# genome/pindel

Hardware: AMD Instinct MI355X
Metric: one-end-anchored reads/sec through split-read search (close end + far end) (higher is better)
Workload: dtype u64; 1 GPU; BASELINE configs[2]: synthetic 10000000 x 100 bp one-end-anchored reads on a chr20-shaped reference (62435964 bp), all SV types (D/SI/TD/INV/none), Pindel defaults -x 2 -a 1 -m 3 -u 0.02 -e 0.01 -E 0.95 -H 8; reads_per_gpu=10000000, reads_total=10000000, read_len=100, insert_size=500, parallelism=reads sharded over 1 GPU(s) (weak scaling), reference replicated, no collective

## Files before the change

pindel_amd/csrc/pg_kernels.hip:

```cpp
#include <hip/hip_runtime.h>
#include <stdint.h>
#include <stdlib.h>

#include "pg_device.h"
#include "pg_lane_masks.h"
#include "pg_eval_masks.h"

typedef unsigned long long u64;
typedef unsigned int u32;
typedef u32 u32x4 __attribute__((ext_vector_type(4)));
typedef u32 u32x8 __attribute__((ext_vector_type(8)));

struct PgKArgs { PgDevRef ref; PgDevParams prm; PgDevBatch B; uint32_t max_len, levels; };
template <typename T> struct KaGlobal { static __device__ __forceinline__ T of(unsigned long long v) { return (T)v; } };
template <typename E> struct KaGlobal<E *> {
    static __device__ __forceinline__ E *of(unsigned long long v) { return (E *)(__attribute__((address_space(1))) E *)v; }
};
template <typename T>
__device__ __forceinline__ T karg_load(int off)
{
    const auto k = __builtin_amdgcn_kernarg_segment_ptr();
    if (sizeof(T) == 8) {
        unsigned long long v;
        asm volatile("s_load_dwordx2 %0, %1, %2\n\ts_waitcnt lgkmcnt(0)" : "=&s"(v) : "s"(k), "n"(off));
        return KaGlobal<T>::of(v);
    } else {
        unsigned int v;
        asm volatile("s_load_dword %0, %1, %2\n\ts_waitcnt lgkmcnt(0)" : "=&s"(v) : "s"(k), "n"(off));
        return (T)v;
    }
}
template <int OFF, typename T>
__device__ __forceinline__ void karg_load3(T &a, T &b, T &c)
{
    static_assert(sizeof(T) == 8, "pointers");
    const auto k = __builtin_amdgcn_kernarg_segment_ptr();
    unsigned long long x, y, z;
    asm volatile("s_load_dwordx2 %0, %3, %4\n\ts_load_dwordx2 %1, %3, %5\n\ts_load_dwordx2 %2, %3, %6\n\ts_waitcnt lgkmcnt(0)"
                 : "=&s"(x), "=&s"(y), "=&s"(z) : "s"(k), "n"(OFF), "n"(OFF + 8), "n"(OFF + 16));
    a = KaGlobal<T>::of(x); b = KaGlobal<T>::of(y); c = KaGlobal<T>::of(z);
}
#define KA(obj, member) karg_load<decltype(obj.member)>((int)offsetof(PgKArgs, obj.member))
#define KAP(member) karg_load<decltype(PgDevParams::member)>((int)offsetof(PgKArgs, prm.member))
#define PRM(member, dflt) (DEF ? (decltype(PgDevParams::member))(dflt) : KA(prm, member))
#define PG_DEF_MAX_RANGE_INDEX 2
#define PG_DEF_ADD_MM 1
#define PG_DEF_MIN_PERFECT 3
#define PG_DEF_MIN_CLOSE 8
#define PG_DEF_SPACER 100000u

#define WAVE 64
#define PG_N_XCD 8u
#define PG_WAVES(NB, Id) (sizeof(Lds<NB, Id>) <= 5120 ? 7 : (sizeof(Lds<NB, Id>) <= 6400 ? 6 : (sizeof(Lds<NB, Id>) <= 7680 ? 5 : 4)))
#define PG_BIG 0xffffu
#define PG_CHR_TAB 24
#define PG_PASS(nb) ((nb) >= 3 ? 32 : 64)
#define PG_CHR_TAB_N(nb) ((nb) >= 3 ? 0 : PG_CHR_TAB)
#define PG_MM_IN_WIN(nb) ((nb) <= 4)

__device__ __forceinline__ u64 ballot64(bool p) { return __builtin_amdgcn_ballot_w64(p); }
__device__ __forceinline__ bool lane_bit(u64 m) { return __builtin_amdgcn_inverse_ballot_w64(m); }
template <int N>
__device__ __forceinline__ u32 row_shr(u32 v)
{
    return (u32)__builtin_amdgcn_update_dpp(0, (int)v, 0x110 + N, 0xf, 0xf, true);
}
__device__ __forceinline__ u32 wave_shr1(u32 v)
{
    return (u32)__builtin_amdgcn_update_dpp(0, (int)v, 0x138, 0xf, 0xf, true);
}
__device__ __forceinline__ u64 wave_shr1(u64 v)
{
    return (u64)wave_shr1((u32)v) | ((u64)wave_shr1((u32)(v >> 32)) << 32);
}
__device__ __forceinline__ u32 wave_scan(u32 v)
{
    v += row_shr<1>(v);
    v += row_shr<2>(v);
    v += row_shr<4>(v);
    v += row_shr<8>(v);
    v += (u32)__builtin_amdgcn_update_dpp(0, (int)v, 0x142, 0xa, 0xf, false);
    v += (u32)__builtin_amdgcn_update_dpp(0, (int)v, 0x143, 0xc, 0xf, false);
    return v;
}
__device__ __forceinline__ u32 read_lane(u32 v, int l) { return (u32)__builtin_amdgcn_readlane((int)v, l); }
__device__ __forceinline__ u64 read_lane(u64 v, int l)
{
    return (u64)read_lane((u32)v, l) | ((u64)read_lane((u32)(v >> 32), l) << 32);
}

#define PG_SYNC()                                              \
    do {                                                       \
        __builtin_amdgcn_fence(__ATOMIC_RELEASE, "wavefront"); \
        __builtin_amdgcn_wave_barrier();                       \
        __builtin_amdgcn_fence(__ATOMIC_ACQUIRE, "wavefront"); \
    } while (0)
__device__ __forceinline__ int uni(int v) { return __builtin_amdgcn_readfirstlane(v); }
__device__ __forceinline__ int opaque(int v)
{
    asm volatile("" : "+v"(v));
    return v;
}
__device__ __forceinline__ int lane_now()
{
    return (int)__builtin_amdgcn_mbcnt_hi(~0u, __builtin_amdgcn_mbcnt_lo(~0u, (u32)opaque(0)));
}
__device__ __forceinline__ u64 low_bits(int n)
{
    return n >= 64 ? ~0ull : (n <= 0 ? 0ull : ((1ull << n) - 1ull));
}
__device__ __forceinline__ u32 low32(int n)
{
    return n >= 32 ? 0xffffffffu : (n <= 0 ? 0u : ((1u << n) - 1u));
}
__device__ __forceinline__ u32 low32_lane(int n)
{
    int t;
    asm("v_med3_i32 %0, %1, 0, 32" : "=v"(t) : "v"(n));
    u32 m;
    asm("v_bfm_b32 %0, %1, 0" : "=v"(m) : "v"(t));
    return m | (0u - ((u32)t >> 5));
}
__device__ __forceinline__ u32 low32_lane4(int n)
{
    int t, f;
    asm("v_med3_i32 %0, %1, 0, 32" : "=v"(t) : "v"(n));
    u32 m;
    asm("v_bfm_b32 %0, %1, 0" : "=v"(m) : "v"(t));
    asm("v_bfe_i32 %0, %1, 5, 1" : "=v"(f) : "v"(t));
    return m | (u32)f;
}
__device__ __forceinline__ u64 low_bits_lane(int n)
{
    return (u64)low32_lane4(n) | ((u64)low32_lane4(n - 32) << 32);
}
template <int NB, int NS, int mode, bool DEF, bool EXACT, int LEN>
constexpr bool pg_short_masks()
{
    if (!DEF || EXACT) return false;
    return !((NB == 4 && NS == 3 && mode == PG_MODE_FAR) || (NB == 8 && NS == 3 && mode == PG_MODE_CLOSE));
}
template <int NB, int NS, typename Id, int mode, bool DEF, bool EXACT, int LEN>
constexpr bool pg_short_eval()
{
    if (!DEF || EXACT) return false;
    if (LEN > 0) return true;
    return (NB == 3 && mode == PG_MODE_FAR) || (NB == 4 && NS == 4 && mode == PG_MODE_BOTH) || (NB == 8 && mode == PG_MODE_CLOSE);
}
__device__ __forceinline__ int count_below(u64 m)
{
    return (int)__builtin_amdgcn_mbcnt_hi((u32)(m >> 32), __builtin_amdgcn_mbcnt_lo((u32)m, 0u));
}
__device__ __forceinline__ u64 bit_range(int lo, int hi)
{
    return low_bits(hi) & ~low_bits(lo);
}
__device__ __forceinline__ u64 funnel64(u32 w0, u32 w1, u32 w2, u32 s)
{
    u32 a = __builtin_amdgcn_alignbit(w1, w0, s);
    u32 b = __builtin_amdgcn_alignbit(w2, w1, s);
    return (u64)a | ((u64)b << 32);
}
__device__ __forceinline__ u32 med3(u32 a, u32 b, u32 c)
{
    u32 r;
    asm("v_med3_u32 %0, %1, %2, %3" : "=v"(r) : "v"(a), "v"(b), "v"(c));
    return r;
}

template <int SHIFT, typename T>
__device__ __forceinline__ T *record_ptr(T *base, uint32_t rid)
{
    const u64 b = (u64)(uintptr_t)base;
    const u32 blo = (u32)uni((int)(u32)b), bhi = (u32)uni((int)(u32)(b >> 32)), r = (u32)uni((int)rid);
    u32 lo, hi;
    asm("s_lshl_b32 %0, %4, %5\n\ts_lshr_b32 %1, %4, %6\n\ts_add_u32 %0, %0, %2\n\ts_addc_u32 %1, %1, %3"
        : "=&s"(lo), "=&s"(hi) : "s"(blo), "s"(bhi), "s"(r), "n"(SHIFT), "n"(32 - SHIFT) : "scc");
    return KaGlobal<T *>::of((u64)lo | ((u64)hi << 32));
}

template <typename Id> struct IdFmt;
template <> struct IdFmt<u32> { static constexpr int RB = PG_REL_BITS_SMALL; };
template <> struct IdFmt<u64> { static constexpr int RB = PG_REL_BITS; };
template <typename Id>
__device__ __forceinline__ Id make_id(u32 rel, bool isB, u32 region)
{
    return (Id)rel | ((Id)(isB ? 1u : 0u) << IdFmt<Id>::RB) | ((Id)region << (IdFmt<Id>::RB + 1));
}

enum { QP_LO = 0, QP_HI = 1, QP_NN = 2, QP_OO = 3 };

template <int NB>
struct Query {
    const u64 *qp;
    bool allowF_, allowB_;
    bool cF_, cB_;
    bool first_ok_;
    bool o1_;
    __device__ __forceinline__ bool allowF() const { return allowF_; }
    __device__ __forceinline__ bool allowB() const { return allowB_; }
    __device__ __forceinline__ bool cF() const { return cF_; }
    __device__ __forceinline__ bool cB() const { return cB_; }
    __device__ __forceinline__ bool first_ok() const { return first_ok_; }
};
template <int NB> __device__ __forceinline__ u64 q_lo(const Query<NB> &Q, int b) { return Q.qp[QP_LO * NB + b]; }
template <int NB> __device__ __forceinline__ u64 q_hi(const Query<NB> &Q, int b) { return Q.qp[QP_HI * NB + b]; }
template <int NB> __device__ __forceinline__ u64 q_nn(const Query<NB> &Q, int b) { return Q.qp[QP_NN * NB + b]; }
template <int NB> __device__ __forceinline__ u64 q_oo(const Query<NB> &Q, int b) { return Q.qp[QP_OO * NB + b]; }

template <typename Id> struct AccB;
template <> struct AccB<u32> {
    typedef uint2 T;
    static __device__ __forceinline__ void load(const void *base, int i, u32 &m1, u32 &m2, u32 &ok, u32 &id)
    {
        const uint2 st = ((const uint2 *)base)[i];
        m1 = st.x & 0xffffu; m2 = (st.x >> 16) & 0x7fffu; ok = st.x >> 31; id = st.y;
    }
    static __device__ __forceinline__ void store(void *base, int i, u32 m1, u32 m2, u32 ok, u32 id)
    {
        const u32 c2 = m2 < 0x7fffu ? m2 : 0x7fffu;
        ((uint2 *)base)[i] = make_uint2(m1 | (c2 << 16) | (ok << 31), id);
    }
};
template <> struct AccB<u64> {
    typedef uint4 T;
    static __device__ __forceinline__ void load(const void *base, int i, u32 &m1, u32 &m2, u32 &ok, u64 &id)
    {
        const uint4 st = ((const uint4 *)base)[i];
        m1 = st.x; m2 = st.y & 0xffffu; ok = st.y >> 16; id = (u64)st.z | ((u64)st.w << 32);
    }
    static __device__ __forceinline__ void store(void *base, int i, u32 m1, u32 m2, u32 ok, u64 id)
    {
        ((uint4 *)base)[i] = make_uint4(m1, m2 | (ok << 16), (u32)id, (u32)(id >> 32));
    }
};

template <int NB, typename Id>
struct Lds {
    uint4 bufA[68];
    uint2 bufB[PG_PASS(NB) * NB];
    uint2 hdrB[64];
    u64 ringB[3 * NB];
    typename AccB<Id>::T accB[NB > 1 ? 64 * (NB - 1) : 1];
    u64 qp[2 * 4 * NB];
    uint16_t queue[PG_PASS(NB)];
    uint8_t mm_tab[PG_MM_IN_WIN(NB) ? 4 : 64 * NB + 64];
    uint2 chr_tab[PG_CHR_TAB_N(NB)];
#ifdef PG_TIMING
    u64 t_last;
    u32 t_acc[12];
    u32 t_pad[2];
#endif
    uint4 win[PG_WIN_STATIC_WORDS(NB)];
};

struct Search {
    int len, T, M, add_mm, bps, min_perfect, thr;
    uint16_t *queue;
    uint4 *win;
    uint4 *bufA;
    uint2 *bufB;
    uint2 *hdrB;
    u64 *ringB;
    void *accB;
    const uint8_t *mm_tab;
    const uint2 *chr_tab;
    u32 depth, jmask[2];
    u32 ro;
    u32 rid;
    u32 rp_lo, rp_hi;
    long long win_wo;
    int win_lo, win_hi, wbase;
    int nsurv;
    u32 nsurv_total;
#ifdef PG_TIMING
    u64 *t_last;
    u32 *t_acc;
    int t_base;
#define PG_T(S, k) do { if (threadIdx.x == 0) { const u64 t_ = __builtin_readcyclecounter(); (S).t_acc[k] += (u32)(t_ - *(S).t_last); *(S).t_last = t_; } } while (0)
#else
#define PG_T(S, k) ((void)0)
#endif
#ifdef PG_STOP
    u32 stopped;
#define PG_STOP_AT(S, k) do { asm volatile("s_nop 14\n\ts_nop %0\n\ts_nop %1" : : "n"((k) & 7), "n"((k) >> 3)); \
                              if (PG_STOP == (k) && uni(opaque(1))) { (S).stopped = 1u; return; } } while (0)
#define PG_STOPPED(S) do { if ((S).stopped) return; } while (0)
#define PG_STOP_AT_V(S, k, v) do { asm volatile("s_nop 14\n\ts_nop %0\n\ts_nop %1" : : "n"((k) & 7), "n"((k) >> 3)); \
                                 if (PG_STOP == (k) && uni(opaque(1))) { (S).stopped = 1u; return (v); } } while (0)
#define PG_STOPPED_V(S, v) do { if ((S).stopped) return (v); } while (0)
#else
#define PG_STOP_AT(S, k) ((void)0)
#define PG_STOPPED(S) ((void)0)
#define PG_STOP_AT_V(S, k, v) ((void)0)
#define PG_STOPPED_V(S, v) ((void)0)
#endif
#ifdef PG_DIAG
    u32 dg;
#endif
#if defined(PG_DIAG) && PG_DIAG == 2
#define PG_DG(S, sh) ((void)0)
#define PG_DC(S, sh) ((S).dg += 1u << (sh))
#define PG_DC_IF(S, cond, sh) ((S).dg += (cond) ? 1u << (sh) : 0u)
#elif defined(PG_DIAG)
#define PG_DG(S, sh) ((S).dg += 1u << (sh))
#define PG_DC(S, sh) ((void)0)
#define PG_DC_IF(S, cond, sh) ((void)0)
#else
#define PG_DG(S, sh) ((void)0)
#define PG_DC(S, sh) ((void)0)
#define PG_DC_IF(S, cond, sh) ((void)0)
#endif
    int cap_state;
    u32 sf;
    __device__ __forceinline__ bool want_cap() const { return (sf & 1u) != 0u; }
    __device__ __forceinline__ bool tierA() const { return (sf & 2u) != 0u; }
    __device__ __forceinline__ bool len_check() const { return (sf & 4u) != 0u; }
};

template <int NB, typename Id>
struct Acc {
    u32 m1, m2, ok;
    Id id;
    u32 a1, a2, aok;
    Id aid;
    u32 dirty;
    __device__ __forceinline__ void reset()
    {
        m1 = m2 = PG_BIG; ok = 0u; id = 0;
        a1 = a2 = PG_BIG; aok = 0u; aid = 0;
        dirty = 0u;
    }
};

template <typename Id>
__device__ __forceinline__ void fold(u32 &m1, u32 &m2, Id &id, u32 &ok, u32 k, Id cid, u32 okc)
{
    const bool lt = k < m1;
    m2 = med3(m1, m2, k);
    id = lt ? cid : id;
    ok = lt ? okc : ok;
    m1 = k < m1 ? k : m1;
}
template <typename Id>
__device__ __forceinline__ void merge(u32 &a1, u32 &a2, Id &aid, u32 &aok, u32 b1, u32 b2, Id bid, u32 bok)
{
    const bool lt = b1 < a1;
    const u32 hi1 = a1 > b1 ? a1 : b1, lo2 = a2 < b2 ? a2 : b2;
    a2 = hi1 < lo2 ? hi1 : lo2;
    aid = lt ? bid : aid;
    aok = lt ? bok : aok;
    a1 = lt ? b1 : a1;
}

__device__ __forceinline__ int max_mismatch_at(const u32 *mm_bp, int L)
{
    int m = 0;
#pragma unroll
    for (int k = 0; k < PG_MM_BREAKS; k++) m += (u32)L >= mm_bp[k] ? 1 : 0;
    return m;
}

template <int NB>
__device__ __forceinline__ long long chr_word_off_of(const PgDevRef &ref, const Search &S, int c)
{
    if (c < PG_CHR_TAB_N(NB)) {
        const uint2 e = S.chr_tab[c];
        if (uni((int)e.y) != 0) return (long long)(u64)(u32)uni((int)e.x);
    }
    const u64 w = KA(ref, chr_word_off)[c];
    return (long long)((u64)(u32)uni((int)(u32)w) | ((u64)(u32)uni((int)(u32)(w >> 32)) << 32));
}
template <int NB>
__device__ __forceinline__ int chr_size_of(const PgDevRef &ref, const Search &S, int c)
{
    if (c < PG_CHR_TAB_N(NB)) {
        const int sz = uni((int)S.chr_tab[c].y);
        if (sz != 0) return sz;
    }
    return uni((int)KA(ref, chr_size)[c]);
}

template <int NB>
__device__ __forceinline__ void block_masks(const Query<NB> &Q, int b, bool comp,
                                            u64 rlo, u64 rhi, u64 rnn, u64 &mis, u64 &qn)
{
    const u64 qlo = q_lo<NB>(Q, b), qhi = q_hi<NB>(Q, b), qnn = q_nn<NB>(Q, b), qoo = q_oo<NB>(Q, b);
    u64 cm = comp ? ~0ull : 0ull;
    u64 x = rlo ^ qlo ^ cm;
    u64 y = rhi ^ qhi ^ cm;
    u64 d = x | y;
    mis = (d & ~qnn) | rnn | qoo;
    qn = qnn;
}

__device__ __forceinline__ void fetch_lds(const uint4 *win, int wbase, int q, bool rev,
                                          u64 &rlo, u64 &rhi, u64 &rnn)
{
    u32 rel = (u32)(q - wbase);
    u32 wi = rel >> 5, s = rel & 31u;
    uint4 w0 = win[wi], w1 = win[wi + 1], w2 = win[wi + 2];
    rlo = funnel64(w0.x, w1.x, w2.x, s);
    rhi = funnel64(w0.y, w1.y, w2.y, s);
    rnn = funnel64(w0.z, w1.z, w2.z, s);
    if (rev) { rlo = __brevll(rlo); rhi = __brevll(rhi); rnn = __brevll(rnn); }
}
__device__ __forceinline__ void fetch_lds_uniform(const uint4 *win, int wbase, int q, bool rev,
                                                  u64 &rlo, u64 &rhi, u64 &rnn)
{
    u32 rel = (u32)(q - wbase);
    u32 wi = rel >> 5, s = rel & 31u;
    uint4 w0 = win[wi], w1 = win[wi + 1], w2 = win[wi + 2];
    rlo = funnel64(w0.x, w1.x, w2.x, s);
    rhi = funnel64(w0.y, w1.y, w2.y, s);
    rnn = funnel64(w0.z, w1.z, w2.z, s);
    if (uni((int)rev)) {
        asm volatile("" : "+v"(rlo), "+v"(rhi), "+v"(rnn));
        rlo = __brevll(rlo); rhi = __brevll(rhi); rnn = __brevll(rnn);
    }
}

struct Rings {
    bool on;
    int s0, e0, s1, e1;
};

template <int NB, typename Id, bool SM>
__device__ __forceinline__ void fold_tier_b(const Search &S, const Query<NB> &Q, Acc<NB, Id> &A, const u64 *longm, int lane)
{
    constexpr int EW = NB;
    {
        u64 any = 0ull;
#pragma unroll
        for (int r = 0; r < NB; r++) any |= longm[r];
        if (any == 0ull) return;
    }
    const int lB = opaque(lane);
    u64 W0, W1, BP0, BP1, BPm;
    if (SM) {
        const PgFoldMasksB k = pg_fold_masks_b(S.bps, S.min_perfect, lB);
        W0 = k.w0; W1 = k.w1; BP0 = k.bp0; BP1 = k.bp1; BPm = 0ull;
    } else {
        const int n0 = S.bps + lB, p0 = n0 - S.min_perfect;
        W0 = low_bits_lane(n0); W1 = low_bits_lane(n0 - 64);
        BP0 = W0 & ~low_bits_lane(p0); BP1 = W1 & ~low_bits_lane(p0 - 64); BPm = ~low_bits_lane(p0 + 64);
    }
#pragma unroll
    for (int r = 0; r < NB; r++) {
        const int L0 = S.bps + 64 * r;
        if (L0 > S.len - 1) break;
        u64 mask = longm[r];
        if (mask == 0ull) continue;
        const int L = L0 + lB;
        u64 Mk[NB], BP[NB], QN[NB];
#pragma unroll
        for (int b = 0; b < NB; b++) {
            Mk[b] = b == r ? W0 : (b == r + 1 ? W1 : ~0ull);
            BP[b] = b == r ? BP0 : (b == r + 1 ? BP1 : BPm);
            QN[b] = q_nn<NB>(Q, b);
        }
        u32 m1 = A.m1, m2 = A.m2, ok = A.ok;
        Id wid = A.id;
        if (r > 0) {
            m1 = m2 = PG_BIG; ok = 0u; wid = 0;
            if ((A.dirty >> r) & 1u) {
                AccB<Id>::load(S.accB, (r - 1) * 64 + lB, m1, m2, ok, wid);
            }
        }
        while (mask != 0ull) {
            const int i = __ffsll((long long)mask) - 1;
            mask &= mask - 1ull;
            const uint2 *e = S.bufB + i * EW;
            const uint2 h = S.hdrB[i];
            u32 k = 0u;
            u64 bad = 0ull;
#pragma unroll
            for (int b = 0; b < NB; b++) {
                if (b > r + 1) continue;
                const uint2 w = e[b];
                const u64 m = (u64)w.x | ((u64)w.y << 32);
                k += (u32)__popcll(b < r ? m : (m & Mk[b]));
                if (b + 1 >= r) bad |= (m ^ QN[b]) & BP[b];
            }
            u32 okc = bad == 0ull ? (h.y >> 31) : 0u;
            if (S.len_check()) okc = (u32)L >= ((h.y >> 24) & 0x7fu) ? okc : 0u;
            const Id cid = sizeof(Id) == 8 ? (Id)((u64)h.x | ((u64)(h.y & 0xffffffu) << 32)) : (Id)h.x;
            fold<Id>(m1, m2, wid, ok, k, cid, okc);
        }
        if (r == 0) { A.m1 = m1; A.m2 = m2; A.ok = ok; A.id = wid; }
        else {
            AccB<Id>::store(S.accB, (r - 1) * 64 + lB, m1, m2, ok, wid);
            A.dirty |= 1u << r;
        }
    }
}

template <int NB, typename Id, bool MIXED, bool SM>
__device__ __forceinline__ void fold_candidates(const Search &S, const Query<NB> &Q, Acc<NB, Id> &A, int wbase,
                                                int origin, u32 region, int n, int lane, const Rings &R, int *ring_n)
{
    constexpr int EW = NB;
    PG_DG(const_cast<Search &>(S), 16);
    const u64 inm = low_bits(n);
    int p = 0;
    bool isB = MIXED ? false : Q.allowB();
    if (lane_bit(inm)) {
        u32 e = S.queue[lane];
        if (MIXED) isB = e & 1u;
        p = wbase + (int)(e >> 1);
    }
    const bool comp = isB ? Q.cB() : Q.cF();
    int cum = 0, lvl0 = 0, kA = 0;
    int kk[NB];
    u32 m0lo = 0u, s0lo = 0u;
#pragma unroll
    for (int r = 0; r < NB; r++) kk[r] = 0;
    u64 needm = inm;
    const int alive = S.T > S.thr ? S.T : S.thr;
#pragma unroll
    for (int b = 0; b < NB; b++) {
        if (64 * b >= S.len) break;
        if (needm == 0ull) break;
        if (lane_bit(needm)) {
            u64 rlo, rhi, rnn, m, s;
            int q = isB ? p - 64 * b - 63 : p + 64 * b;
            if (MIXED) fetch_lds(S.win, wbase, q, isB, rlo, rhi, rnn);
            else fetch_lds_uniform(S.win, wbase, q, isB, rlo, rhi, rnn);
            block_masks<NB>(Q, b, comp, rlo, rhi, rnn, m, s);
            const u64 lm = low_bits(S.len - 64 * b);
            m &= lm;
            s = (m ^ s) & lm;
            S.bufB[lane * EW + b] = make_uint2((u32)m, (u32)(m >> 32));
            cum += __popcll(m);
            if (b == 0) {
                lvl0 = __popcll(m & low_bits(S.bps));
                kA = __popc((u32)m & low32(S.bps + 16));
                m0lo = (u32)m;
                s0lo = (u32)s;
            }
#pragma unroll
            for (int r = 1; r < NB; r++)
                if (b <= r) kk[r] += __popcll(m & low_bits(S.bps + 64 * r - 64 * b));
        }
        needm &= ballot64(cum < alive);
    }
    const u32 hamok = cum >= S.thr ? 0x80000000u : 0u;
    const u64 validm = inm & ballot64(lvl0 < S.T);
    u64 lngm = validm;
    if (S.tierA()) lngm &= ballot64(kA < S.T);
    const bool lng = lane_bit(lngm);
    const Id id = make_id<Id>((u32)(p - origin), isB, region);
    const u32 lenthr = (u32)(S.min_perfect + (isB ? 0 : 1));
    const u32 meta = (u32)((u64)id >> 32) | (lenthr << 24) | hamok;
    const u64 shortm = validm & ~lngm;
    const bool sht = lane_bit(shortm);
    u64 longm[NB];
    const int nA = __popcll(shortm);
    int qb, qs, qe, n_iter;
    {
        const int qd = opaque(lane) >> 4;
        if (MIXED && R.on) {
            const u32 w0 = R.e0 > R.s0 ? (u32)(R.e0 - R.s0) : 0u, w1 = R.e1 > R.s1 ? (u32)(R.e1 - R.s1) : 0u;
            const u64 in0 = inm & ballot64((u32)(p - R.s0) < w0);
            const u64 in1 = inm & ~in0 & ballot64((u32)(p - R.s1) < w1);
            const int ring = lane_bit(in0) ? 0 : (lane_bit(in1) ? 1 : 2);
            ring_n[0] = __popcll(in0);
            ring_n[1] = __popcll(in1);
            ring_n[2] = n - ring_n[0] - ring_n[1];
            const u64 sh0 = shortm & in0, sh1 = shortm & in1, sh2 = shortm & ~(in0 | in1);
            const int n0 = __popcll(sh0), n1 = __popcll(sh1), n2 = nA - n0 - n1;
            if (sht) {
                const u64 mine = ring == 0 ? sh0 : (ring == 1 ? sh1 : sh2);
                const int rank = count_below(mine) + (ring == 0 ? 0 : (ring == 1 ? n0 : n0 + n1));
                S.bufA[rank] = make_uint4(m0lo, s0lo, (u32)id, meta);
            }
            qb = qd == 0 ? 0 : (qd == 1 ? n0 : n0 + n1 + (qd - 2));
            qs = qd < 2 ? 1 : 2;
            qe = qd == 0 ? n0 : (qd == 1 ? n0 + n1 : nA);
            const int h2 = (n2 + 1) >> 1;
            n_iter = n0 > n1 ? n0 : n1;
            n_iter = n_iter > h2 ? n_iter : h2;
            const u64 inl[3] = { in0, in1, ~(in0 | in1) };
#pragma unroll
            for (int x = 0; x < 3; x++) {
                const u64 l0 = lngm & inl[x];
                if (lane == 0) S.ringB[x * NB] = l0;
#pragma unroll
                for (int r = 1; r < NB; r++) {
                    const u64 lr = lngm & ballot64(kk[r] < S.T) & inl[x];
                    if (lane == 0) S.ringB[x * NB + r] = lr;
                }
            }
        } else {
            if (sht) {
                const int rank = count_below(shortm);
                S.bufA[rank] = make_uint4(m0lo, s0lo, (u32)id, meta);
            }
            qb = qd;
            qs = 4;
            qe = nA;
            n_iter = (nA + 3) >> 2;
            longm[0] = lngm;
#pragma unroll
            for (int r = 1; r < NB; r++) longm[r] = lngm & ballot64(kk[r] < S.T);
        }
    }
    if (lng) S.hdrB[lane] = make_uint2((u32)id, meta);
    PG_STOP_AT(const_cast<Search &>(S), (MIXED && R.on) ? 28 : 17);
    PG_SYNC();
    if (nA > 0) {
        const int lA = opaque(lane);
        u32 mk, bpm;
        if (SM) {
            const PgFoldMasksA k = pg_fold_masks_a(S.bps, S.min_perfect, lA);
            mk = k.mk; bpm = k.bpm;
        } else {
            const int L = S.bps + (lA & 15);
            mk = low32_lane(L);
            bpm = mk & ~low32_lane(L - S.min_perfect);
        }
        int idx = qb;
        for (int it = 0; it < n_iter; it++, idx += qs) {
            const uint4 e = S.bufA[idx < 67 ? idx : 67];
            u32 k = (u32)__popc(e.x & mk);
            k = idx < qe ? k : PG_BIG;
            const u32 okc = (e.y & bpm) == 0u ? (e.w >> 31) : 0u;
            const Id cid = sizeof(Id) == 8 ? (Id)((u64)e.z | ((u64)(e.w & 0xffffffu) << 32)) : (Id)e.z;
            fold<Id>(A.a1, A.a2, A.aid, A.aok, k, cid, okc);
        }
    }
    if (!(MIXED && R.on)) fold_tier_b<NB, Id, SM>(S, Q, A, longm, lane);
    PG_SYNC();
    PG_STOP_AT(const_cast<Search &>(S), (MIXED && R.on) ? 29 : 18);
}

template <int NB, bool WIDE = false>
__device__ __forceinline__ void stage_window(const PgDevRef &ref, Search &S, long long wo, int lo, int hi, int lane,
                                             const PgInRec *next_rec = nullptr)
{
    const int nw = ((hi - lo + 31) >> 5) + 2;
    const u32 sh = (u32)(lo & 31);
    PG_DG(S, 0);
    PG_SYNC();
    {
        const long long g0 = wo + (long long)(lo >> 5);
        const u32 *glo, *ghi, *gnn;
        karg_load3<(int)offsetof(PgKArgs, ref.lo)>(glo, ghi, gnn);
        glo += g0; ghi += g0; gnn += g0;
        if (WIDE && nw > 2 * WAVE) {
            const int i = lane, j = lane + WAVE, k = lane + 2 * WAVE;
            const bool three = k < nw;
            const u32 oi = 4u * (u32)i, oj = 4u * (u32)j, ok = 4u * (u32)(three ? k : i);
            u64 a, b, c, d, e, f, g, h, m;
            asm volatile("global_load_dwordx2 %0, %9, %12\n\tglobal_load_dwordx2 %1, %9, %13\n\tglobal_load_dwordx2 %2, %9, %14\n\t"
                         "global_load_dwordx2 %3, %10, %12\n\tglobal_load_dwordx2 %4, %10, %13\n\tglobal_load_dwordx2 %5, %10, %14\n\t"
                         "global_load_dwordx2 %6, %11, %12\n\tglobal_load_dwordx2 %7, %11, %13\n\tglobal_load_dwordx2 %8, %11, %14\n\t"
                         "s_waitcnt vmcnt(0)"
                         : "=&v"(a), "=&v"(b), "=&v"(c), "=&v"(d), "=&v"(e), "=&v"(f), "=&v"(g), "=&v"(h), "=&v"(m)
                         : "v"(oi), "v"(oj), "v"(ok), "s"(glo), "s"(ghi), "s"(gnn) : "memory");
            *(uint3 *)__builtin_assume_aligned(&S.win[i], 16) =
                make_uint3(__builtin_amdgcn_alignbit((u32)(a >> 32), (u32)a, sh), __builtin_amdgcn_alignbit((u32)(b >> 32), (u32)b, sh),
                           __builtin_amdgcn_alignbit((u32)(c >> 32), (u32)c, sh));
            *(uint3 *)__builtin_assume_aligned(&S.win[j], 16) =
                make_uint3(__builtin_amdgcn_alignbit((u32)(d >> 32), (u32)d, sh), __builtin_amdgcn_alignbit((u32)(e >> 32), (u32)e, sh),
                           __builtin_amdgcn_alignbit((u32)(f >> 32), (u32)f, sh));
            if (three)
                *(uint3 *)__builtin_assume_aligned(&S.win[k], 16) =
                    make_uint3(__builtin_amdgcn_alignbit((u32)(g >> 32), (u32)g, sh), __builtin_amdgcn_alignbit((u32)(h >> 32), (u32)h, sh),
                               __builtin_amdgcn_alignbit((u32)(m >> 32), (u32)m, sh));
        } else
        for (int i = lane; i < nw; i += 2 * WAVE) {
            const int j = i + WAVE;
            const bool two = j < nw;
            const u32 oi = 4u * (u32)i, oj = 4u * (u32)(two ? j : i);
            u64 a, b, c, d, e, f;
            if (next_rec) {
                u32 touched;
                asm volatile("global_load_dwordx2 %[a], %[oi], %[glo]\n\tglobal_load_dwordx2 %[b], %[oi], %[ghi]\n\tglobal_load_dwordx2 %[c], %[oi], %[gnn]\n\t"
                             "global_load_dwordx2 %[d], %[oj], %[glo]\n\tglobal_load_dwordx2 %[e], %[oj], %[ghi]\n\tglobal_load_dwordx2 %[f], %[oj], %[gnn]\n\t"
                             "s_load_dword %[t], %[nr], 0x0\n\t"
                             "s_waitcnt vmcnt(0) lgkmcnt(0)"
                             : [a] "=&v"(a), [b] "=&v"(b), [c] "=&v"(c), [d] "=&v"(d), [e] "=&v"(e), [f] "=&v"(f), [t] "=&s"(touched)
                             : [oi] "v"(oi), [oj] "v"(oj), [glo] "s"(glo), [ghi] "s"(ghi), [gnn] "s"(gnn), [nr] "s"(next_rec) : "memory");
            } else
            asm volatile("global_load_dwordx2 %0, %6, %8\n\tglobal_load_dwordx2 %1, %6, %9\n\tglobal_load_dwordx2 %2, %6, %10\n\t"
                         "global_load_dwordx2 %3, %7, %8\n\tglobal_load_dwordx2 %4, %7, %9\n\tglobal_load_dwordx2 %5, %7, %10\n\t"
                         "s_waitcnt vmcnt(0)"
                         : "=&v"(a), "=&v"(b), "=&v"(c), "=&v"(d), "=&v"(e), "=&v"(f)
                         : "v"(oi), "v"(oj), "s"(glo), "s"(ghi), "s"(gnn) : "memory");
            *(uint3 *)__builtin_assume_aligned(&S.win[i], 16) =
                make_uint3(__builtin_amdgcn_alignbit((u32)(a >> 32), (u32)a, sh), __builtin_amdgcn_alignbit((u32)(b >> 32), (u32)b, sh),
                           __builtin_amdgcn_alignbit((u32)(c >> 32), (u32)c, sh));
            if (two)
                *(uint3 *)__builtin_assume_aligned(&S.win[j], 16) =
                    make_uint3(__builtin_amdgcn_alignbit((u32)(d >> 32), (u32)d, sh), __builtin_amdgcn_alignbit((u32)(e >> 32), (u32)e, sh),
                               __builtin_amdgcn_alignbit((u32)(f >> 32), (u32)f, sh));
        }
    }
    PG_SYNC();
    S.win_wo = wo;
    S.wbase = lo;
    S.win_lo = lo;
    S.win_hi = hi;
}

__device__ __forceinline__ u32 bits32(int lo, int hi)
{
    return low32(hi) & ~low32(lo);
}


__host__ __device__ constexpr u32 le3_table(int t)
{
    u32 tt = 0u;
    for (int i = 0; i < 8; i++) {
        const int v = 4 * (i & 1) + 2 * ((i >> 1) & 1) + ((i >> 2) & 1);
        if (v <= t) tt |= 1u << i;
    }
    return tt;
}
#define PG_BO3(a, b, c, tt) __builtin_amdgcn_bitop3_b32((a), (b), (c), (tt))
template <int NS, bool TWO>
__device__ __forceinline__ void count_le(const u32 *c, u32 ov, const u32 *d, u32 ovd, int thr, u32 &rc, u32 &rd)
{
    thr = uni(thr);
    rd = 0u;
    if (thr < 0) { rc = 0u; return; }
    if (thr >= (1 << NS) - 1) { rc = ~ov; if (TWO) rd = ~ovd; return; }
    u32 g, h = 0u;
#define PG_LE3(t) g = PG_BO3(c[0], c[1], c[2], le3_table(t)); if (TWO) h = PG_BO3(d[0], d[1], d[2], le3_table(t)); break;
    switch (thr & 7) {
    case 0: PG_LE3(0)
    case 1: PG_LE3(1)
    case 2: PG_LE3(2)
    case 3: PG_LE3(3)
    case 4: PG_LE3(4)
    case 5: PG_LE3(5)
    case 6: PG_LE3(6)
    default: g = h = ~0u; break;
    }
#undef PG_LE3
    if (NS == 3) {
        rc = PG_BO3(g, ov, ov, 0x30);
        if (TWO) rd = PG_BO3(h, ovd, ovd, 0x30);
    } else if (NS == 4) {
        if (thr >> 3) {
            rc = PG_BO3(g, c[3], ov, 0x51);
            if (TWO) rd = PG_BO3(h, d[3], ovd, 0x51);
        } else {
            rc = PG_BO3(g, c[3], ov, 0x10);
            if (TWO) rd = PG_BO3(h, d[3], ovd, 0x10);
        }
    } else {
        u32 u, v = 0u;
#define PG_LE5(tt) u = PG_BO3(g, c[3], c[4], tt); if (TWO) v = PG_BO3(h, d[3], d[4], tt); break;
        switch (thr >> 3) {
        case 0: PG_LE5(0x10)
        case 1: PG_LE5(0x51)
        case 2: PG_LE5(0x75)
        default: PG_LE5(0xf7)
        }
#undef PG_LE5
        rc = PG_BO3(u, ov, ov, 0x30);
        if (TWO) rd = PG_BO3(v, ovd, ovd, 0x30);
    }
}

#define PG_TAKE(j) "s_ff1_i32_b32 %[" j "], %[pm]\n\ts_bitset0_b32 %[pm], %[" j "]\n\t"
#define PG_SHIFT(m, j) "v_alignbit_b32 %[" m "], %[hi], %[lo], %[" j "]\n\t"
#define PG_MIRROR(t, j) "s_sub_i32 %[" t "], 32, %[" j "]\n\t"
#define PG_ADD1 "v_bitop3_b32 %[k0], %[ma], %[c0], %[c0] bitop3:0x0c\n\tv_bitop3_b32 %[c0], %[c0], %[ma], %[ma] bitop3:0xc3\n\t" \
                "v_and_b32 %[k1], %[c1], %[k0]\n\tv_xor_b32 %[c1], %[c1], %[k0]\n\t"
#define PG_ADD2 "v_bitop3_b32 %[k0], %[c0], %[ma], %[mb] bitop3:0x60\n\tv_bitop3_b32 %[c0], %[c0], %[ma], %[mb] bitop3:0x96\n\t" \
                "v_bitop3_b32 %[s0], %[ma], %[mb], %[k0] bitop3:0xab\n\t" \
                "v_and_b32 %[k1], %[c1], %[s0]\n\tv_xor_b32 %[c1], %[c1], %[s0]\n\t"
#define PG_ADD3 "v_bitop3_b32 %[s0], %[ma], %[mb], %[mc] bitop3:0x69\n\tv_bitop3_b32 %[s1], %[ma], %[mb], %[mc] bitop3:0x17\n\t" \
                "v_and_b32 %[k0], %[c0], %[s0]\n\tv_xor_b32 %[c0], %[c0], %[s0]\n\t" \
                "v_bitop3_b32 %[k1], %[c1], %[s1], %[k0] bitop3:0xe8\n\tv_bitop3_b32 %[c1], %[c1], %[s1], %[k0] bitop3:0x96\n\t"
#define PG_UP3 "v_bitop3_b32 %[ov], %[c2], %[k1], %[ov] bitop3:0xea\n\tv_xor_b32 %[c2], %[c2], %[k1]"
#define PG_UP4 "v_and_b32 %[k0], %[c2], %[k1]\n\tv_xor_b32 %[c2], %[c2], %[k1]\n\t" \
               "v_bitop3_b32 %[ov], %[c3], %[k0], %[ov] bitop3:0xea\n\tv_xor_b32 %[c3], %[c3], %[k0]"
#define PG_UP5 "v_and_b32 %[k0], %[c2], %[k1]\n\tv_xor_b32 %[c2], %[c2], %[k1]\n\t" \
               "v_and_b32 %[k1], %[c3], %[k0]\n\tv_xor_b32 %[c3], %[c3], %[k0]\n\t" \
               "v_bitop3_b32 %[ov], %[c4], %[k1], %[ov] bitop3:0xea\n\tv_xor_b32 %[c4], %[c4], %[k1]"
template <int NS>
struct Counter {
    u32 c0, c1, c2, c3, c4, ov;
    __device__ __forceinline__ void reset() { c0 = c1 = c2 = c3 = c4 = ov = 0u; }
    template <bool TWO>
    __device__ __forceinline__ void le(const Counter &o, int thr, u32 &mine, u32 &others) const
    {
        const u32 c[5] = { c0, c1, c2, c3, c4 }, d[5] = { o.c0, o.c1, o.c2, o.c3, o.c4 };
        count_le<NS, TWO>(c, ov, d, o.ov, thr, mine, others);
    }
#define PG_CTR3 [c0] "+v"(c0), [c1] "+v"(c1), [c2] "+v"(c2), [ov] "+v"(ov)
#define PG_CTR4 [c0] "+v"(c0), [c1] "+v"(c1), [c2] "+v"(c2), [c3] "+v"(c3), [ov] "+v"(ov)
#define PG_CTR5 [c0] "+v"(c0), [c1] "+v"(c1), [c2] "+v"(c2), [c3] "+v"(c3), [c4] "+v"(c4), [ov] "+v"(ov)
#define PG_PLANES [lo] "v"(lo), [hi] "v"(hi)
    __device__ __forceinline__ void take1(u32 &pm, u32 lo, u32 hi, u32 &ja)
    {
        u32 ma, k0, k1;
        if (NS == 3)
            asm(PG_TAKE("ja") PG_SHIFT("ma", "ja") PG_ADD1 PG_UP3
                : PG_CTR3, [pm] "+s"(pm), [ja] "=&s"(ja), [ma] "=&v"(ma), [k0] "=&v"(k0), [k1] "=&v"(k1) : PG_PLANES);
        else if (NS == 4)
            asm(PG_TAKE("ja") PG_SHIFT("ma", "ja") PG_ADD1 PG_UP4
                : PG_CTR4, [pm] "+s"(pm), [ja] "=&s"(ja), [ma] "=&v"(ma), [k0] "=&v"(k0), [k1] "=&v"(k1) : PG_PLANES);
        else
            asm(PG_TAKE("ja") PG_SHIFT("ma", "ja") PG_ADD1 PG_UP5
                : PG_CTR5, [pm] "+s"(pm), [ja] "=&s"(ja), [ma] "=&v"(ma), [k0] "=&v"(k0), [k1] "=&v"(k1) : PG_PLANES);
    }
    __device__ __forceinline__ void take2(u32 &pm, u32 lo, u32 hi, u32 &ja, u32 &jb)
    {
        u32 ma, mb, s0, k0, k1;
        if (NS == 3)
            asm(PG_TAKE("ja") PG_TAKE("jb") PG_SHIFT("ma", "ja") PG_SHIFT("mb", "jb") PG_ADD2 PG_UP3
                : PG_CTR3, [pm] "+s"(pm), [ja] "=&s"(ja), [jb] "=&s"(jb), [ma] "=&v"(ma), [mb] "=&v"(mb), [s0] "=&v"(s0),
                  [k0] "=&v"(k0), [k1] "=&v"(k1) : PG_PLANES);
        else if (NS == 4)
            asm(PG_TAKE("ja") PG_TAKE("jb") PG_SHIFT("ma", "ja") PG_SHIFT("mb", "jb") PG_ADD2 PG_UP4
                : PG_CTR4, [pm] "+s"(pm), [ja] "=&s"(ja), [jb] "=&s"(jb), [ma] "=&v"(ma), [mb] "=&v"(mb), [s0] "=&v"(s0),
                  [k0] "=&v"(k0), [k1] "=&v"(k1) : PG_PLANES);
        else
            asm(PG_TAKE("ja") PG_TAKE("jb") PG_SHIFT("ma", "ja") PG_SHIFT("mb", "jb") PG_ADD2 PG_UP5
                : PG_CTR5, [pm] "+s"(pm), [ja] "=&s"(ja), [jb] "=&s"(jb), [ma] "=&v"(ma), [mb] "=&v"(mb), [s0] "=&v"(s0),
                  [k0] "=&v"(k0), [k1] "=&v"(k1) : PG_PLANES);
    }
    __device__ __forceinline__ void take3(u32 &pm, u32 lo, u32 hi, u32 &ja, u32 &jb, u32 &jc)
    {
        u32 ma, mb, mc, s0, s1, k0, k1;
        if (NS == 3)
            asm(PG_TAKE("ja") PG_TAKE("jb") PG_TAKE("jc") PG_SHIFT("ma", "ja") PG_SHIFT("mb", "jb") PG_SHIFT("mc", "jc")
                PG_ADD3 PG_UP3
                : PG_CTR3, [pm] "+s"(pm), [ja] "=&s"(ja), [jb] "=&s"(jb), [jc] "=&s"(jc), [ma] "=&v"(ma), [mb] "=&v"(mb),
                  [mc] "=&v"(mc), [s0] "=&v"(s0), [s1] "=&v"(s1), [k0] "=&v"(k0), [k1] "=&v"(k1) : PG_PLANES);
        else if (NS == 4)
            asm(PG_TAKE("ja") PG_TAKE("jb") PG_TAKE("jc") PG_SHIFT("ma", "ja") PG_SHIFT("mb", "jb") PG_SHIFT("mc", "jc")
                PG_ADD3 PG_UP4
                : PG_CTR4, [pm] "+s"(pm), [ja] "=&s"(ja), [jb] "=&s"(jb), [jc] "=&s"(jc), [ma] "=&v"(ma), [mb] "=&v"(mb),
                  [mc] "=&v"(mc), [s0] "=&v"(s0), [s1] "=&v"(s1), [k0] "=&v"(k0), [k1] "=&v"(k1) : PG_PLANES);
        else
            asm(PG_TAKE("ja") PG_TAKE("jb") PG_TAKE("jc") PG_SHIFT("ma", "ja") PG_SHIFT("mb", "jb") PG_SHIFT("mc", "jc")
                PG_ADD3 PG_UP5
                : PG_CTR5, [pm] "+s"(pm), [ja] "=&s"(ja), [jb] "=&s"(jb), [jc] "=&s"(jc), [ma] "=&v"(ma), [mb] "=&v"(mb),
                  [mc] "=&v"(mc), [s0] "=&v"(s0), [s1] "=&v"(s1), [k0] "=&v"(k0), [k1] "=&v"(k1) : PG_PLANES);
    }
    __device__ __forceinline__ void mirror1(u32 lo, u32 hi, u32 ja)
    {
        u32 ta, ma, k0, k1;
        if (NS == 3)
            asm(PG_MIRROR("ta", "ja") PG_SHIFT("ma", "ta") PG_ADD1 PG_UP3
                : PG_CTR3, [ta] "=&s"(ta), [ma] "=&v"(ma), [k0] "=&v"(k0), [k1] "=&v"(k1) : PG_PLANES, [ja] "s"(ja) : "scc");
        else if (NS == 4)
            asm(PG_MIRROR("ta", "ja") PG_SHIFT("ma", "ta") PG_ADD1 PG_UP4
                : PG_CTR4, [ta] "=&s"(ta), [ma] "=&v"(ma), [k0] "=&v"(k0), [k1] "=&v"(k1) : PG_PLANES, [ja] "s"(ja) : "scc");
        else
            asm(PG_MIRROR("ta", "ja") PG_SHIFT("ma", "ta") PG_ADD1 PG_UP5
                : PG_CTR5, [ta] "=&s"(ta), [ma] "=&v"(ma), [k0] "=&v"(k0), [k1] "=&v"(k1) : PG_PLANES, [ja] "s"(ja) : "scc");
    }
    __device__ __forceinline__ void mirror2(u32 lo, u32 hi, u32 ja, u32 jb)
    {
        u32 ta, tb, ma, mb, s0, k0, k1;
        if (NS == 3)
            asm(PG_MIRROR("ta", "ja") PG_MIRROR("tb", "jb") PG_SHIFT("ma", "ta") PG_SHIFT("mb", "tb") PG_ADD2 PG_UP3
                : PG_CTR3, [ta] "=&s"(ta), [tb] "=&s"(tb), [ma] "=&v"(ma), [mb] "=&v"(mb), [s0] "=&v"(s0), [k0] "=&v"(k0),
                  [k1] "=&v"(k1) : PG_PLANES, [ja] "s"(ja), [jb] "s"(jb) : "scc");
        else if (NS == 4)
            asm(PG_MIRROR("ta", "ja") PG_MIRROR("tb", "jb") PG_SHIFT("ma", "ta") PG_SHIFT("mb", "tb") PG_ADD2 PG_UP4
                : PG_CTR4, [ta] "=&s"(ta), [tb] "=&s"(tb), [ma] "=&v"(ma), [mb] "=&v"(mb), [s0] "=&v"(s0), [k0] "=&v"(k0),
                  [k1] "=&v"(k1) : PG_PLANES, [ja] "s"(ja), [jb] "s"(jb) : "scc");
        else
            asm(PG_MIRROR("ta", "ja") PG_MIRROR("tb", "jb") PG_SHIFT("ma", "ta") PG_SHIFT("mb", "tb") PG_ADD2 PG_UP5
                : PG_CTR5, [ta] "=&s"(ta), [tb] "=&s"(tb), [ma] "=&v"(ma), [mb] "=&v"(mb), [s0] "=&v"(s0), [k0] "=&v"(k0),
                  [k1] "=&v"(k1) : PG_PLANES, [ja] "s"(ja), [jb] "s"(jb) : "scc");
    }
    __device__ __forceinline__ void mirror3(u32 lo, u32 hi, u32 ja, u32 jb, u32 jc)
    {
        u32 ta, tb, tc, ma, mb, mc, s0, s1, k0, k1;
        if (NS == 3)
            asm(PG_MIRROR("ta", "ja") PG_MIRROR("tb", "jb") PG_MIRROR("tc", "jc") PG_SHIFT("ma", "ta") PG_SHIFT("mb", "tb")
                PG_SHIFT("mc", "tc") PG_ADD3 PG_UP3
                : PG_CTR3, [ta] "=&s"(ta), [tb] "=&s"(tb), [tc] "=&s"(tc), [ma] "=&v"(ma), [mb] "=&v"(mb), [mc] "=&v"(mc),
                  [s0] "=&v"(s0), [s1] "=&v"(s1), [k0] "=&v"(k0), [k1] "=&v"(k1) : PG_PLANES, [ja] "s"(ja), [jb] "s"(jb), [jc] "s"(jc) : "scc");
        else if (NS == 4)
            asm(PG_MIRROR("ta", "ja") PG_MIRROR("tb", "jb") PG_MIRROR("tc", "jc") PG_SHIFT("ma", "ta") PG_SHIFT("mb", "tb")
                PG_SHIFT("mc", "tc") PG_ADD3 PG_UP4
                : PG_CTR4, [ta] "=&s"(ta), [tb] "=&s"(tb), [tc] "=&s"(tc), [ma] "=&v"(ma), [mb] "=&v"(mb), [mc] "=&v"(mc),
                  [s0] "=&v"(s0), [s1] "=&v"(s1), [k0] "=&v"(k0), [k1] "=&v"(k1) : PG_PLANES, [ja] "s"(ja), [jb] "s"(jb), [jc] "s"(jc) : "scc");
        else
            asm(PG_MIRROR("ta", "ja") PG_MIRROR("tb", "jb") PG_MIRROR("tc", "jc") PG_SHIFT("ma", "ta") PG_SHIFT("mb", "tb")
                PG_SHIFT("mc", "tc") PG_ADD3 PG_UP5
                : PG_CTR5, [ta] "=&s"(ta), [tb] "=&s"(tb), [tc] "=&s"(tc), [ma] "=&v"(ma), [mb] "=&v"(mb), [mc] "=&v"(mc),
                  [s0] "=&v"(s0), [s1] "=&v"(s1), [k0] "=&v"(k0), [k1] "=&v"(k1) : PG_PLANES, [ja] "s"(ja), [jb] "s"(jb), [jc] "s"(jc) : "scc");
    }
};

template <int NS, bool DUAL>
__device__ __forceinline__ void add_bases(bool group, u32 pm, Counter<NS> &C, u32 lo, u32 hi,
                                          Counter<NS> &C2, u32 lo2, u32 hi2)
{
    u32 ja, jb, jc;
    if (group) {
        int n = __popc(pm);
        while (n >= 3) {
            C.take3(pm, lo, hi, ja, jb, jc);
            if (DUAL) C2.mirror3(lo2, hi2, ja, jb, jc);
            n -= 3;
        }
        if (n == 2) {
            C.take2(pm, lo, hi, ja, jb);
            if (DUAL) C2.mirror2(lo2, hi2, ja, jb);
        }
    }
    while (pm != 0u) {
        C.take1(pm, lo, hi, ja);
        if (DUAL) C2.mirror1(lo2, hi2, ja);
    }
}

template <int NB, int NS, bool DUAL>
__device__ __forceinline__ void seed_filter_run(const Search &S, const Query<NB> &Q, bool kindB, int lane,
                                                u32 jmask, u32 g0mask, int cap0, u32 &mF, u32 &mB)
{
    u32 lo = (u32)uni((int)(u32)q_lo<NB>(Q, 0)), hi = (u32)uni((int)(u32)q_hi<NB>(Q, 0));
    const u32 nn = (u32)uni((int)(u32)q_nn<NB>(Q, 0)), oo = (u32)uni((int)(u32)q_oo<NB>(Q, 0));
    if (DUAL ? Q.cF() : (kindB ? Q.cB() : Q.cF())) { lo = ~lo; hi = ~hi; }
    const u32 acgt = ~(nn | oo);
    const u32 sym[5] = { ~lo & ~hi & acgt, lo & ~hi & acgt, ~lo & hi & acgt, lo & hi & acgt, nn };
    const int a = 2 * NB + lane;
    const bool useF = DUAL || !kindB, useB = DUAL || kindB;
    const uint4 p0 = S.win[a];
    u32 w0[5], w1[5], wm[5];
    w0[0] = ~(p0.x | p0.y | p0.z);
    w0[1] = p0.x & ~(p0.y | p0.z);
    w0[2] = p0.y & ~(p0.x | p0.z);
    w0[3] = p0.x & p0.y & ~p0.z;
    w0[4] = ~p0.z;
#pragma unroll
    for (int X = 0; X < 5; X++) w1[X] = wm[X] = 0u;
    if (useF) {
        const uint4 p1 = S.win[a + 1];
        w1[0] = ~(p1.x | p1.y | p1.z);
        w1[1] = p1.x & ~(p1.y | p1.z);
        w1[2] = p1.y & ~(p1.x | p1.z);
        w1[3] = p1.x & p1.y & ~p1.z;
        w1[4] = ~p1.z;
    }
    if (useB) {
        const uint4 pm1 = S.win[a - 1];
        wm[0] = ~(pm1.x | pm1.y | pm1.z);
        wm[1] = pm1.x & ~(pm1.y | pm1.z);
        wm[2] = pm1.y & ~(pm1.x | pm1.z);
        wm[3] = pm1.x & pm1.y & ~pm1.z;
        wm[4] = ~pm1.z;
    }
    const u32 l0 = (lo & 1u) ? ~0u : 0u, h0 = (hi & 1u) ? ~0u : 0u;
    const u32 seed = ~((p0.x ^ l0) | (p0.y ^ h0) | p0.z);
    const u32 seed2 = ~((p0.x ^ ~l0) | (p0.y ^ ~h0) | p0.z);
    const int o_pre = __popc(oo & g0mask), o_all = __popc(oo & jmask);
    Counter<NS> C, C2;
    C.reset();
    C2.reset();
    u32 snap = 0u, snap2 = 0u;
#pragma unroll
    for (int it = 0; it < 10; it++) {
        const int X = it >= 5 ? it - 5 : it;
        const int X2 = X < 4 ? 3 - X : X;
        if (it == 5) C.template le<DUAL>(C2, cap0 - o_pre, snap, snap2);
        u32 pm = sym[X] & (it >= 5 ? (jmask & ~g0mask) : g0mask);
        if (DUAL) add_bases<NS, true>(X < 4, pm, C, w0[X], w1[X], C2, wm[X2], w0[X2]);
        else if (kindB) add_bases<NS, false>(X < 4, __brev(pm) << 1, C, wm[X], w0[X], C2, 0u, 0u);
        else add_bases<NS, false>(X < 4, pm, C, w0[X], w1[X], C2, 0u, 0u);
    }
    u32 fin, fin2;
    C.template le<DUAL>(C2, S.T - 1 - o_all, fin, fin2);
    mF = seed & (snap | fin);
    if (DUAL) mB = seed2 & (snap2 | fin2);
}

#define RO_ONEHOT(dA, dC, dG, dT, dN, x, y, z)                                                                       \
    "v_bitop3_b32 " dA ", " x ", " y ", " z " bitop3:0x01\n\tv_bitop3_b32 " dC ", " x ", " y ", " z " bitop3:0x10\n\t" \
    "v_bitop3_b32 " dG ", " x ", " y ", " z " bitop3:0x04\n\tv_bitop3_b32 " dT ", " x ", " y ", " z " bitop3:0x40\n\t" \
    "v_not_b32 " dN ", " z "\n\t"
#define RO_ADD3_CORE(c0, c1, ma, mb, mc)                                                                              \
    "v_bitop3_b32 v35, " ma ", " mb ", " mc " bitop3:0x69\n\tv_bitop3_b32 v36, " ma ", " mb ", " mc " bitop3:0x17\n\t"   \
    "v_and_b32 v37, " c0 ", v35\n\tv_xor_b32 " c0 ", " c0 ", v35\n\t"                                                   \
    "v_bitop3_b32 v38, " c1 ", v36, v37 bitop3:0xe8\n\tv_bitop3_b32 " c1 ", " c1 ", v36, v37 bitop3:0x96\n\t"
#define RO_UP3(c2, ov) "v_bitop3_b32 " ov ", " c2 ", v38, " ov " bitop3:0xea\n\tv_xor_b32 " c2 ", " c2 ", v38\n\t"
#define RO_UP4(c2, c3, ov) "v_and_b32 v37, " c2 ", v38\n\tv_xor_b32 " c2 ", " c2 ", v38\n\t"                            \
                           "v_bitop3_b32 " ov ", " c3 ", v37, " ov " bitop3:0xea\n\tv_xor_b32 " c3 ", " c3 ", v37\n\t"
#ifndef RO_IDX_ON
#define RO_IDX_ON(P) "s_set_gpr_idx_on " P ", 0x3\n\t"
#define RO_IDX_1(P) "s_bfe_u32 m0, " P ", 0x100008\n\t"
#define RO_IDX_2(P) "s_bfe_u32 m0, " P ", 0x100010\n\t"
#define RO_IDX_OFF "s_set_gpr_idx_off\n\t"
#endif
#define RO_SH(P, s1, s2, s3)                                                                                           \
    RO_IDX_ON(P) "v_alignbit_b32 v32, v5, v0, " #s1 "\n\t"                                                              \
    RO_IDX_1(P) "v_alignbit_b32 v33, v5, v0, " #s2 "\n\t"                                                               \
    RO_IDX_2(P) "v_alignbit_b32 v34, v5, v0, " #s3 "\n\t" RO_IDX_OFF
#define RO_AD3 RO_ADD3_CORE("v40", "v41", "v32", "v33", "v34") RO_UP3("v42", "v43")
#define RO_AD4 RO_ADD3_CORE("v40", "v41", "v32", "v33", "v34") RO_UP4("v42", "v44", "v43")
#define RO_PROG_LOAD "s_load_dwordx4 s[84:87], %[rp], %[off]\n\t"
#define RO_PROG_LOAD2 "s_load_dwordx4 s[84:87], %[rp], %[off] offset:0x10\n\t"
#define RO_SH_F(P, j1, j2, j3, n1, n2, n3) RO_SH(P, j1, j2, j3)
#define RO_SH_B(P, j1, j2, j3, n1, n2, n3) RO_SH(P, n1, n2, n3)
#define RO_G1(M) M("s84", 1, 2, 3, 31, 30, 29)
#define RO_G2(M) M("s85", 4, 5, 6, 28, 27, 26)
#define RO_G3(M) M("s86", 7, 8, 9, 25, 24, 23)
#define RO_G4(M) M("s87", 10, 11, 12, 22, 21, 20)
#define RO_G5(M) M("s84", 13, 14, 15, 19, 18, 17)
#define RO_G6(M) M("s85", 16, 17, 18, 16, 15, 14)
#define RO_G7(M) M("s86", 19, 20, 21, 13, 12, 11)
#define RO_G8(M) M("s87", 22, 23, 24, 10, 9, 8)
#define RO_EXIT(k) "s_cmp_eq_u32 %[G], " #k "\n\ts_cbranch_scc1 9f\n\t"
#define RO_INIT3 "v_bfe_i32 v40, %[t], 0, 1\n\tv_bfe_i32 v41, %[t], 1, 1\n\tv_bfe_i32 v42, %[t], 2, 1\n\tv_mov_b32 v43, 0\n\t"
#define RO_INIT4 RO_INIT3 "v_bfe_i32 v44, %[t], 3, 1\n\t"
#define RO_DMASK3 "v_bfe_i32 v35, %[t], 4, 1\n\tv_bfe_i32 v36, %[t], 5, 1\n\tv_bfe_i32 v37, %[t], 6, 1\n\t"
#define RO_DMASK4 RO_DMASK3 "v_bfe_i32 v45, %[t], 7, 1\n\t"
#define RO_CARRY0 "v_and_b32 v38, v40, v35\n\t"
#define RO_CARRY1 "v_bitop3_b32 v38, v40, v35, v32 bitop3:0xd4\n\t"
#define RO_REST3 "v_bitop3_b32 v38, v41, v36, v38 bitop3:0xe8\n\tv_bitop3_b32 v38, v42, v37, v38 bitop3:0xe8\n\t" \
                 "v_bitop3_b32 v39, v38, v43, v43 bitop3:0x01\n\t"
#define RO_REST4 "v_bitop3_b32 v38, v41, v36, v38 bitop3:0xe8\n\tv_bitop3_b32 v38, v42, v37, v38 bitop3:0xe8\n\t" \
                 "v_bitop3_b32 v38, v44, v45, v38 bitop3:0xe8\n\tv_bitop3_b32 v39, v38, v43, v43 bitop3:0x01\n\t"
#define RO_TAIL(SH, AD) RO_G4(SH) RO_PROG_LOAD2 AD RO_EXIT(4) "s_waitcnt lgkmcnt(0)\n\t"                                \
    RO_G5(SH) AD RO_EXIT(5) RO_G6(SH) AD RO_EXIT(6) RO_G7(SH) AD RO_EXIT(7) RO_G8(SH) AD
#define RO_RUN_CLOSE(SH, AD, DM, RS) RO_G1(SH) AD RO_G2(SH) AD RO_G3(SH) DM RO_CARRY1 RS AD RO_TAIL(SH, AD)
#define RO_RUN_FAR(SH, AD, DM, RS) RO_G1(SH) AD RO_G2(SH) AD RO_G3(SH) AD DM RO_CARRY0 RS RO_TAIL(SH, AD)
#define RO_FINAL(SEEDREG) "9:\n\ts_waitcnt lgkmcnt(0)\n\ts_set_gpr_idx_on s88, 0x1\n\tv_mov_b32 v32, " SEEDREG "\n\ts_set_gpr_idx_off\n\t" \
                          "v_bitop3_b32 %[m], v32, v39, v43 bitop3:0xd0"
#define RO_CLOBBERS4 "v44", "v45",
#define RO_CLOBBERS "v32", "v33", "v34", "v35", "v36", "v37", "v38", "v39", "v40", "v41", "v42", "v43",                   \
                    "v48", "v49", "v50", "v51", "v52", "v53", "v54", "v55", "v56", "v57",                               \
                    "s84", "s85", "s86", "s87", "s88", "m0", "scc", "memory"
template <int NB, int KIND, bool FAR, int NS>
__device__ __forceinline__ u32 seed_filter_ro1(const Search &S, bool o1, bool wide, int word)
{
    static_assert(NS == 3 || NS == 4, "three slices (up to 8 mismatch levels) or four (up to 16)");
    const u32 ro = S.ro;
    const u32 G = (ro >> (wide ? 4 : 0)) & 15u;
    const int bound = (int)((ro >> (wide ? 16 : 8)) & 0xffu);
    const int thrA = bound < S.cap_state ? bound : S.cap_state;
    const u32 t = (u32)((1 << NS) - S.T) | ((u32)(S.T - 1 - thrA) << 4);
    const u32 off = o1 ? 0x60u : 0x40u;
    const u32 wa = (u32)(uintptr_t)(const __attribute__((address_space(3))) uint4 *)(S.win + (2 * NB + word - (KIND == 1 ? 1 : 0)));
    const PgInRec *rp = KaGlobal<const PgInRec *>::of((u64)S.rp_lo | ((u64)S.rp_hi << 32));
    u32 m;
#define RO_HEAD(INIT) RO_PROG_LOAD "ds_read_b128 v[32:35], %[wa]\n\tds_read_b128 v[36:39], %[wa] offset:16\n\t" INIT "s_waitcnt lgkmcnt(0)\n\ts_lshr_b32 s88, s84, 24\n\t"
#define RO_OPERANDS(MORE) : [m] "=&v"(m) : [rp] "s"(rp), [off] "s"(off), [wa] "v"(wa), [t] "s"(t), [G] "s"(G) : MORE RO_CLOBBERS
#define RO_PLANES_F RO_ONEHOT("v48", "v49", "v50", "v51", "v52", "v32", "v33", "v34") RO_ONEHOT("v53", "v54", "v55", "v56", "v57", "v36", "v37", "v38")
#define RO_PLANES_B RO_ONEHOT("v51", "v50", "v49", "v48", "v52", "v32", "v33", "v34") RO_ONEHOT("v56", "v55", "v54", "v53", "v57", "v36", "v37", "v38")
    if (NS == 3) {
        if (KIND == 0 && FAR) asm volatile(RO_HEAD(RO_INIT3) RO_PLANES_F RO_RUN_FAR(RO_SH_F, RO_AD3, RO_DMASK3, RO_REST3) RO_FINAL("v0") RO_OPERANDS());
        else if (KIND == 0) asm volatile(RO_HEAD(RO_INIT3) RO_PLANES_F RO_RUN_CLOSE(RO_SH_F, RO_AD3, RO_DMASK3, RO_REST3) RO_FINAL("v0") RO_OPERANDS());
        else if (FAR) asm volatile(RO_HEAD(RO_INIT3) RO_PLANES_B RO_RUN_FAR(RO_SH_B, RO_AD3, RO_DMASK3, RO_REST3) RO_FINAL("v5") RO_OPERANDS());
        else asm volatile(RO_HEAD(RO_INIT3) RO_PLANES_B RO_RUN_CLOSE(RO_SH_B, RO_AD3, RO_DMASK3, RO_REST3) RO_FINAL("v5") RO_OPERANDS());
    } else {
        if (KIND == 0 && FAR) asm volatile(RO_HEAD(RO_INIT4) RO_PLANES_F RO_RUN_FAR(RO_SH_F, RO_AD4, RO_DMASK4, RO_REST4) RO_FINAL("v0") RO_OPERANDS(RO_CLOBBERS4));
        else if (KIND == 0) asm volatile(RO_HEAD(RO_INIT4) RO_PLANES_F RO_RUN_CLOSE(RO_SH_F, RO_AD4, RO_DMASK4, RO_REST4) RO_FINAL("v0") RO_OPERANDS(RO_CLOBBERS4));
        else if (FAR) asm volatile(RO_HEAD(RO_INIT4) RO_PLANES_B RO_RUN_FAR(RO_SH_B, RO_AD4, RO_DMASK4, RO_REST4) RO_FINAL("v5") RO_OPERANDS(RO_CLOBBERS4));
        else asm volatile(RO_HEAD(RO_INIT4) RO_PLANES_B RO_RUN_CLOSE(RO_SH_B, RO_AD4, RO_DMASK4, RO_REST4) RO_FINAL("v5") RO_OPERANDS(RO_CLOBBERS4));
    }
    return m;
}
template <int NB, int KIND, int NS = 3>
__device__ __forceinline__ void seed_filter_ro(const Search &S, bool o1, bool wide, int word, u32 &mF, u32 &mB)
{
    if (KIND == 2) {
        mF = seed_filter_ro1<NB, 0, true, NS>(S, o1, wide, word);
        mB = seed_filter_ro1<NB, 1, true, NS>(S, o1, wide, word);
    } else
        mF = seed_filter_ro1<NB, KIND, false, NS>(S, o1, wide, word);
}

template <int NB, int NS, bool DUAL>
__device__ __forceinline__ void seed_filter(const Search &S, const Query<NB> &Q, bool kindB, bool wide, int lane,
                                            u32 &mF, u32 &mB)
{
    const int T = S.T;
    PG_DG(const_cast<Search &>(S), 8);
    if (NS <= 4 && (S.ro & PG_RO_OK)) {
        constexpr int RNS = NS <= 3 ? 3 : 4;
        if (DUAL) seed_filter_ro<NB, 2, RNS>(S, Q.o1_, wide, lane, mF, mB);
        else if (kindB) seed_filter_ro<NB, 1, RNS>(S, Q.o1_, wide, lane, mF, mB);
        else seed_filter_ro<NB, 0, RNS>(S, Q.o1_, wide, lane, mF, mB);
        return;
    }
    const u32 jmask = S.jmask[wide ? 1 : 0];
    const u32 g0mask = jmask & low32(S.bps);
    int cap0 = (int)((S.depth >> (wide ? 24 : 16)) & 0xffu);
    if (cap0 > S.cap_state) cap0 = S.cap_state;
    seed_filter_run<NB, NS, DUAL>(S, Q, kindB, lane, jmask, g0mask, cap0, mF, mB);
}

template <int NB, int NS, typename Id, bool MIXED, bool W3, bool SM>
__device__ __forceinline__ void scan_impl(const PgDevRef &ref, Search &S,
                                          const Query<NB> &Q, Acc<NB, Id> &A, long long wo, int g0, int s, int e,
                                          int e_max, int xs, int xe, int origin, u32 region, int lane,
                                          u32 use_cache, u32 &cacheF, u32 &cacheB, u32 &cache_valid)
{
    if (!Q.first_ok() || s >= e) return;
    PG_STOP_AT(S, 33);
    const int k0 = (s - g0) >> PG_CHUNK_SHIFT, k1 = (e - 1 - g0) >> PG_CHUNK_SHIFT;
    for (int k = k0; k <= k1; k++) {
        const int cs = g0 + (k << PG_CHUNK_SHIFT);
        const int ns = s > cs ? s : cs;
        {
            const int ne = e < cs + (int)PG_CHUNK ? e : cs + (int)PG_CHUNK;
            if (ns >= xs && ne <= xe) continue;
        }
        const int wb = cs - 64 * NB;
        if (MIXED && !(use_cache && k == 0)) {
            int nh = 1;
            const bool pair_ok = PG_PAIR_CHUNKS(NB) && (PG_WIN_DYN_BYTES(NB) == 0u || S.want_cap());
            if (pair_ok && k + 1 <= k1 && !(use_cache && k + 1 == 0)) {
                const int c1 = cs + (int)PG_CHUNK;
                const int ns1 = s > c1 ? s : c1, ne1 = e < c1 + (int)PG_CHUNK ? e : c1 + (int)PG_CHUNK;
                if (!(ns1 >= xs && ne1 <= xe)) nh = 2;
            }
            const int ce = cs + nh * (int)PG_CHUNK;
            const int ne = e < ce ? e : ce;
            const int se = e_max < ce ? e_max : ce;
            if (!(wo == S.win_wo && S.wbase == wb && se + 64 * NB <= S.win_hi))
                stage_window<NB, W3>(ref, S, wo, wb, se + 64 * NB, lane);
            int h = 0, end = 0, slot = 0;
            u32 mF = 0u, mB = 0u, pos0 = 0u;
            for (;;) {
                while (mF != 0u && slot < PG_PASS(NB)) {
                    const int bit = __ffs((int)mF) - 1;
                    mF &= mF - 1u;
                    S.queue[slot] = (uint16_t)((pos0 + (u32)bit) << 1);
                    slot++;
                }
                while (mF == 0u && mB != 0u && slot < PG_PASS(NB)) {
                    const int bit = __ffs((int)mB) - 1;
                    mB &= mB - 1u;
                    S.queue[slot] = (uint16_t)(((pos0 + (u32)bit) << 1) | 1u);
                    slot++;
                }
                int n;
                if (end >= PG_PASS(NB)) n = PG_PASS(NB);
                else if (h < nh) {
                    const int word = 64 * h + lane;
                    seed_filter<NB, NS, true>(S, Q, false, true, word, mF, mB);
                    const int pbase = cs + 32 * word;
                    const u32 rmask = bits32(ns - pbase, ne - pbase) & ~bits32(xs - pbase, xe - pbase);
                    mF &= rmask;
                    mB &= rmask;
                    h++;
                    if (ballot64((mF | mB) != 0u) == 0ull) continue;
                    const u32 cnt = (u32)(__popc(mF) + __popc(mB));
                    const u32 incl = wave_scan(cnt);
                    slot = end + (int)(incl - cnt);
                    end += (int)read_lane(incl, 63);
                    pos0 = (u32)(64 * NB + 32 * word);
                    continue;
                }
                else if (end > 0) n = end;
                else break;
                S.nsurv += n;
                S.nsurv_total += (u32)n;
                PG_SYNC();
                PG_T(S, S.t_base);
                fold_candidates<NB, Id, MIXED, SM>(S, Q, A, wb, origin, region, n, lane, Rings{ false, 0, 0, 0, 0 }, nullptr);
                PG_STOPPED(S);
                PG_T(S, S.t_base + 1);
                slot -= n;
                end -= n;
                if (end == 0 && h == nh) break;
            }
            k += nh - 1;
            continue;
        }
        const int ne = e < cs + (int)PG_CHUNK ? e : cs + (int)PG_CHUNK;
        const int se = e_max < cs + (int)PG_CHUNK ? e_max : cs + (int)PG_CHUNK;
        PG_STOP_AT(S, 34);
        if (!(wo == S.win_wo && S.wbase == wb && se + 64 * NB <= S.win_hi))
            stage_window<NB>(ref, S, wo, wb, se + 64 * NB, lane);
        PG_STOP_AT(S, 13);
        const int pbase = cs + 32 * lane;
        const u32 rmask = (low32_lane(ne - pbase) & ~low32_lane(ns - pbase)) & ~(low32_lane(xe - pbase) & ~low32_lane(xs - pbase));
        const bool cached = use_cache && k == 0 && cache_valid != 0u;
        u32 mF = 0u, mB = 0u;
        PG_STOP_AT(S, 37);
        if (cached) {
            mF = cacheF;
            mB = cacheB;
        } else {
            if (MIXED) {
                seed_filter<NB, NS, true>(S, Q, false, false, lane, mF, mB);
            } else {
                u32 unused;
                if (Q.allowF()) seed_filter<NB, NS, false>(S, Q, false, false, lane, mF, unused);
                if (Q.allowB()) seed_filter<NB, NS, false>(S, Q, true, false, lane, mB, unused);
            }
            if (use_cache && k == 0) { cacheF = mF; cacheB = mB; }
        }
        PG_STOP_AT(S, 14);
        mF &= rmask;
        mB &= rmask;
        if (use_cache && k == 0) cache_valid = 1u;
        const u32 cnt = (u32)(__popc(mF) + __popc(mB));
        const u32 incl = wave_scan(cnt);
        const int total = (int)read_lane(incl, 63);
        int slot = (int)(incl - cnt);
        PG_STOP_AT(S, 15);
        for (int base = 0; base < total; base += PG_PASS(NB)) {
            PG_SYNC();
            const int top = base + PG_PASS(NB);
            while (mF != 0u && slot < top) {
                const int bit = __ffs((int)mF) - 1;
                mF &= mF - 1u;
                S.queue[slot - base] = (uint16_t)((u32)(64 * NB + 32 * lane + bit) << 1);
                slot++;
            }
            while (mF == 0u && mB != 0u && slot < top) {
                const int bit = __ffs((int)mB) - 1;
                mB &= mB - 1u;
                S.queue[slot - base] = (uint16_t)(((u32)(64 * NB + 32 * lane + bit) << 1) | 1u);
                slot++;
            }
            const int n = total - base < PG_PASS(NB) ? total - base : PG_PASS(NB);
            S.nsurv += n;
            S.nsurv_total += (u32)n;
            PG_SYNC();
            PG_T(S, S.t_base);
            PG_STOP_AT(S, 16);
            fold_candidates<NB, Id, MIXED, SM>(S, Q, A, wb, origin, region, n, lane, Rings{ false, 0, 0, 0, 0 }, nullptr);
            PG_STOPPED(S);
            PG_T(S, S.t_base + 1);
        }
    }
}

template <int NB, int NS, typename Id, bool W3, bool SM>
__device__ __forceinline__ void scan_range(const PgDevRef &ref, Search &S,
                                           const Query<NB> &Q, Acc<NB, Id> &A, long long wo, int g0, int s, int e,
                                           int e_max, int xs, int xe, int origin, u32 region, int lane,
                                           u32 use_cache, u32 &cacheF, u32 &cacheB, u32 &cache_valid)
{
    g0 = uni(g0); s = uni(s); e = uni(e); e_max = uni(e_max); xs = uni(xs); xe = uni(xe); origin = uni(origin);
    if (Q.allowF() && Q.allowB())
        scan_impl<NB, NS, Id, true, W3, SM>(ref, S, Q, A, wo, g0, s, e, e_max, xs, xe, origin, region, lane,
                                    use_cache, cacheF, cacheB, cache_valid);
    else
        scan_impl<NB, NS, Id, false, false, SM>(ref, S, Q, A, wo, g0, s, e, e_max, xs, xe, origin, region, lane,
                                        use_cache, cacheF, cacheB, cache_valid);
}

template <int NB, int NS, typename Id, bool SM>
__device__ __forceinline__ void scan_staged(Search &S, const Query<NB> &Q, Acc<NB, Id> &A, int g0, int s, int e, int origin,
                                            int lane, u32 keep, u32 &cacheF, u32 &cacheB, u32 &cache_valid)
{
    const int wb = g0 - 64 * NB;
    PG_STOP_AT(S, 33);
    PG_STOP_AT(S, 34);
    PG_STOP_AT(S, 13);
    PG_STOP_AT(S, 37);
    u32 mF = 0u, mB = 0u, unused;
    if (Q.allowB()) seed_filter<NB, NS, false>(S, Q, true, false, lane, mB, unused);
    else seed_filter<NB, NS, false>(S, Q, false, false, lane, mF, unused);
    if (keep) { cacheF = mF; cacheB = mB; cache_valid = 1u; }
    PG_STOP_AT(S, 14);
    const u32 kb = Q.allowB() ? 1u : 0u;
    const int pbase = g0 + 32 * lane;
    u32 m = (mF | mB) & low32_lane(e - pbase) & ~low32_lane(s - pbase);
    const u32 cnt = (u32)__popc(m);
    const u32 incl = wave_scan(cnt);
    const int total = (int)read_lane(incl, 63);
    int slot = (int)(incl - cnt);
    PG_STOP_AT(S, 15);
    for (int base = 0; base < total; base += PG_PASS(NB)) {
        PG_SYNC();
        const int top = base + PG_PASS(NB);
        while (m != 0u && slot < top) {
            const int bit = __ffs((int)m) - 1;
            m &= m - 1u;
            S.queue[slot - base] = (uint16_t)(((u32)(64 * NB + 32 * lane + bit) << 1) | kb);
            slot++;
        }
        const int n = total - base < PG_PASS(NB) ? total - base : PG_PASS(NB);
        S.nsurv += n;
        S.nsurv_total += (u32)n;
        PG_SYNC();
        PG_T(S, S.t_base);
        PG_STOP_AT(S, 16);
        fold_candidates<NB, Id, false, SM>(S, Q, A, wb, origin, 0u, n, lane, Rings{ false, 0, 0, 0, 0 }, nullptr);
        PG_STOPPED(S);
        PG_T(S, S.t_base + 1);
    }
}

struct RegionInfo {
    int chr;
    int origin;
    const pg_window *bd;
};

template <int NB, typename Id>
struct Eval {
    Id id[NB];
    u32 lo[NB];
    u64 startm[NB], brkm[NB];
    int n_runs, max_len;
    Id id_last;
};

template <int NB>
__device__ __forceinline__ u32 mm_of(const Search &S, int L)
{
    if (PG_MM_IN_WIN(NB)) return (S.win[L >> 2].w >> (8 * (L & 3))) & 0xffu;
    return S.mm_tab[L];
}

template <int NB, typename Id, bool SE>
__device__ __forceinline__ void evaluate(Search &S, const Acc<NB, Id> &A, Eval<NB, Id> &E, int lane, int qmask = 15)
{
    static_assert(PG_MM_BREAKS < 64, "the short form's reach rule: no level of a point reaches 64");
    const u32 mm0 = mm_of<NB>(S, S.bps + lane);
    E.n_runs = 0;
    E.max_len = 0;
    E.id_last = 0;
    PG_DG(S, 24);
    u32 t1 = A.m1, t2 = A.m2, tok = A.ok;
    Id tid = A.id;
    if (S.tierA()) {
        u32 a1 = PG_BIG, a2 = PG_BIG, aok = 0u;
        Id aid = 0;
        if (lane < 16) { a1 = A.a1; a2 = A.a2; aok = A.aok; aid = A.aid; }
        if (qmask != 1) {
            PG_DC(S, 24);
            S.bufA[lane] = make_uint4(A.a1, A.a2 | (A.aok << 16), (u32)A.aid, (u32)((u64)A.aid >> 32));
            PG_SYNC();
            if (lane < 16) {
#pragma unroll
                for (int q = 1; q < 4; q++) {
                    if (!((qmask >> q) & 1)) continue;
                    const uint4 o = S.bufA[lane + 16 * q];
                    const Id oid = sizeof(Id) == 8 ? (Id)((u64)o.z | ((u64)o.w << 32)) : (Id)o.z;
                    merge<Id>(a1, a2, aid, aok, o.x, o.y & 0xffffu, oid, o.y >> 16);
                }
            }
            PG_SYNC();
        }
        merge<Id>(t1, t2, tid, tok, a1, a2, aid, aok);
    }
    if (S.want_cap()) {
        const int J = (int)((S.depth >> 8) & 0xffu);
        u32 v = (S.bps + lane <= J) ? t1 : 0u;
        u32 o;
        o = row_shr<1>(v); v = v > o ? v : o;
        o = row_shr<2>(v); v = v > o ? v : o;
        o = row_shr<4>(v); v = v > o ? v : o;
        o = row_shr<8>(v); v = v > o ? v : o;
        u32 mx = read_lane(v, 15);
        const u32 m2_ = read_lane(v, 31);
        mx = mx > m2_ ? mx : m2_;
        const int cap = (int)mx + S.add_mm;
        S.cap_state = cap < S.T - 1 ? cap : S.T - 1;
    }
    u32 aborted = 0u;
#pragma unroll
    for (int r = 0; r < NB; r++) {
        E.startm[r] = 0ull;
        E.brkm[r] = ~0ull;
        E.id[r] = 0;
        E.lo[r] = 0u;
        const int r0 = S.bps + 64 * r;
        if (r0 > S.len - 1 || aborted) continue;
        const int L = r0 + lane;
        const bool valid = L <= S.len - 1;
        u32 m1 = t1, m2 = t2, ok = tok, mmL = mm0;
        Id wid = tid;
        if (r > 0) {
            m1 = m2 = PG_BIG; ok = 0u; wid = 0;
            mmL = mm_of<NB>(S, L);
            if ((A.dirty >> r) & 1u) {
                AccB<Id>::load(S.accB, (r - 1) * 64 + lane, m1, m2, ok, wid);
            }
        }
        const u32 lo = m1 <= (u32)S.M ? m1 : (u32)S.M + 1u;
        const u64 vm = SE ? pg_em_valid(S.len, r0) : ballot64(valid);
        const u64 ab = vm & ballot64(lo > mmL);
        u64 cm;
        if (SE) {
            cm = vm & (~ab & (ab - 1ull)) & ballot64(m2 > m1 + (u32)S.add_mm) & ballot64(ok != 0u);
            if (pg_em_reach_needs_compare(r)) cm &= ballot64((u32)lane >= m1);
        } else
            cm = vm & (~ab & (ab - 1ull)) & ballot64(m1 <= (u32)S.M) & ballot64(m2 > m1 + (u32)S.add_mm) &
                 ballot64((u32)L >= (u32)S.bps + m1) & ballot64(ok != 0u);
        PG_DC(S, 12);
        PG_DC_IF(S, cm == 0ull, 16);
        if (SE && cm == 0ull) {
            if (ab) aborted = 1u;
            continue;
        }
        const u32 lok = lane_bit(cm) ? lo + 1u : 0u;
        const u32 plok = wave_shr1(lok);
        u64 samem = ballot64(plok == lok) & ballot64(wave_shr1((u32)wid) == (u32)wid);
        if (sizeof(Id) == 8) samem &= ballot64(wave_shr1((u32)((u64)wid >> 32)) == (u32)((u64)wid >> 32));
        E.id[r] = wid;
        E.lo[r] = lo;
        E.startm[r] = cm & ~samem;
        E.brkm[r] = E.startm[r] | ~cm;
        E.n_runs += __popcll(E.startm[r]);
        if (cm) {
            const int top = 63 - __clzll((long long)cm);
            E.max_len = r0 + top;
            E.id_last = read_lane(wid, top);
        }
        if (ab) aborted = 1u;
    }
    PG_DC_IF(S, E.max_len == 0, 8);
}

template <int NB, typename Id, bool SE>
__device__ __forceinline__ int count_kept(const Eval<NB, Id> &E, bool only_last, u64 *kept)
{
    int n = 0;
#pragma unroll
    for (int r = 0; r < NB; r++) {
        kept[r] = E.startm[r];
        if (only_last && E.startm[r]) kept[r] &= ballot64(E.id[r] == E.id_last);
        n += __popcll(kept[r]);
    }
    return n;
}

template <int NB, typename Id, bool SE>
__device__ __forceinline__ void emit_runs(const Search &S, bool antiF, bool antiB, int chr0, int origin0,
                                          const pg_window *bd, const Eval<NB, Id> &E, const u64 *kept,
                                          pg_run *out, int lane)
{
    typedef IdFmt<Id> F;
    int written = 0;
#pragma unroll
    for (int r = 0; r < NB; r++) {
        if (kept[r] == 0ull) continue;
        if ((kept[r] >> lane) & 1ull) {
            const int L = S.bps + 64 * r + lane;
            const u64 higher = E.brkm[r] & (SE ? pg_em_above(lane) : ~low_bits_lane(lane + 1));
            const int end_lane = higher ? __ffsll((long long)higher) - 2 : WAVE - 1;
            const u64 id = (u64)E.id[r];
            const u32 rel = (u32)(id & ((1ull << F::RB) - 1ull));
            const bool isB = (id >> F::RB) & 1ull;
            int chr = chr0, origin = origin0;
            if (bd) {
                const pg_window w = bd[(u32)(id >> (F::RB + 1))];
                chr = w.chr_id;
                origin = w.start < 0 ? w.end - 1 : w.start;
            }
            const int p = origin + (int)rel;
            const bool anti = isB ? antiB : antiF;
            u32 *dst = (u32 *)(out + written + count_below(kept[r]));
            dst[0] = isB ? (u32)(p - L + 1) : (u32)(p + L - 1);
            dst[1] = (u32)L | ((u32)(S.bps + 64 * r + end_lane) << 16);
            dst[2] = E.lo[r] | ((isB ? PG_RUN_BACKWARD : 0u) << 8) | ((anti ? PG_RUN_ANTISENSE : 0u) << 8) |
                     ((u32)(chr & 0xffff) << 16);
        }
        written += __popcll(kept[r]);
    }
}

template <int NB>
__device__ __forceinline__ u64 request_planes(const PgDevBatch &B, uint32_t rid, int lane)
{
    const u32 pb = KA(B, plane_blocks);
    return (u32)lane < 8u * pb ? KA(B, planes)[(size_t)rid * 8u * pb + (u32)lane] : 0ull;
}
template <int NB>
__device__ __forceinline__ void store_planes(const PgDevBatch &B, u64 v, int lane, u64 *qp)
{
    const u32 pb = KA(B, plane_blocks);
    PG_SYNC();
    if ((u32)lane < 8u * pb) qp[pb == (u32)NB ? (u32)lane : ((u32)lane / pb) * NB + (u32)lane % pb] = v;
    PG_SYNC();
}

__device__ __forceinline__ u32 pool_alloc(const PgDevBatch &B, int n, int lane, u32 &fits)
{
    const u32 shard = blockIdx.x & (PG_POOL_SHARDS - 1u);
    u32 off = 0;
    if (n > 0 && lane == 0) off = atomicAdd(KA(B, pool_used) + shard * 16u, (u32)n);
    off = (u32)uni((int)off);
    fits = (u64)off + (u64)n <= (u64)KA(B, pool_shard_cap) ? 1u : 0u;
    return shard * KA(B, pool_shard_cap) + off;
}

template <int NB, int NS, typename Id, int mode, bool DEF, bool EXACT = false, int LEN = 0>
__device__ __forceinline__ void search_read(const PgDevRef &ref, const PgDevParams &prm, const PgDevBatch &B,
                                            Search &S, u64 *qplanes, const uint32_t rid, const int touch_next, const int lane,
                                            const u32 res_base, const u32 res_fits)
{
#define PG_LANE (NB <= 2 ? lane_now() : opaque(lane))
    S.win_wo = -1;
    S.win_hi = S.wbase = 0;
    S.nsurv_total = 0u;
#ifdef PG_TIMING
    S.t_base = 1;
#endif
#ifdef PG_DIAG
    S.dg = 0u;
#endif
    S.cap_state = 255;
    S.sf = 0u;
#ifdef PG_STOP
    S.stopped = 0u;
#endif
    const u64 planes_of_read = request_planes<NB>(B, rid, lane);
    const PgInRec *rp = record_ptr<7>(KA(B, in), rid);
    u32x8 ra;
    u32x4 rb;
    asm volatile("s_load_dwordx8 %0, %2, 0x0\n\ts_load_dwordx4 %1, %2, 0x20\n\ts_waitcnt lgkmcnt(0)" : "=&s"(ra), "=&s"(rb) : "s"(rp));
    int len = (int)(ra[6] & 0xffffu);
    u32 flags = ra[6] >> 16;
    const int chr = (int)rb[3];
    const long long chr_wo = (long long)((u64)ra[4] | ((u64)ra[5] << 32));
    S.len = len;
    S.thr = (int)(ra[7] & 0xffffu);
    S.M = (int)((ra[7] >> 16) & 0xffu);
    S.T = (int)(ra[7] >> 24);
    S.add_mm = PRM(add_mm, PG_DEF_ADD_MM);
    S.min_perfect = PRM(min_perfect, PG_DEF_MIN_PERFECT);
    static_assert(PG_DEF_MIN_PERFECT <= PG_DEF_MIN_CLOSE && PG_DEF_MIN_PERFECT <= 10, "the short masks need min_perfect <= bps at both ends");
    constexpr bool SM = pg_short_masks<NB, NS, mode, DEF, EXACT, LEN>();
    constexpr bool SE = pg_short_eval<NB, NS, Id, mode, DEF, EXACT, LEN>();
    S.depth = rb[0];
    S.jmask[0] = rb[1];
    S.jmask[1] = 0u;
    S.ro = rb[2];
    if (LEN > 0) {
        static_assert(LEN == 0 || (!EXACT && DEF && mode == PG_MODE_BOTH), "fixed length: the fused default-parameter kernels only");
        constexpr PgFixedLen F = pg_fixed_len_row((uint32_t)LEN);
        static_assert(LEN == 0 || F.len == (uint32_t)LEN, "no baked row for this length");
        len = LEN;
        S.len = LEN;
        S.thr = (int)(F.lvl & 0xffffu);
        S.M = (int)((F.lvl >> 16) & 0xffu);
        S.T = (int)(F.lvl >> 24);
        S.depth = F.depth;
        S.jmask[0] = F.jmask0;
        S.ro = F.ro;
    }
    S.rid = rid;
    S.rp_lo = (u32)uni((int)(u32)(u64)(uintptr_t)rp);
    S.rp_hi = (u32)uni((int)(u32)((u64)(uintptr_t)rp >> 32));
    PG_STOP_AT(S, 10);
    if ((mode & PG_MODE_CLOSE) && (flags & PG_RF_CLOSE_OK)) {
        const int ss = (int)ra[2], se = (int)ra[3];
        if (ss < se) stage_window<NB>(ref, S, chr_wo, ss - 64 * NB, se + 64 * NB, lane, rp + uni(touch_next));
    }
    store_planes<NB>(B, planes_of_read, lane, qplanes);

    PG_T(S, 0);
#if defined(PG_STOP) && PG_STOP == 1
    if (uni(opaque(1))) return;
#endif
    int ja = 0, jb = 0, ex_stage = 0;
    auto ex_apply = [&](int to) __attribute__((always_inline)) {
        while (ex_stage < to) {
            ex_stage++;
            const int cut = ex_stage == 1 ? ja : jb;
            u64 *pl = qplanes + (ex_stage == 1 ? 0 : 4 * NB);
            if (cut > 0) {
                const int l = PG_LANE;
                u64 v = 0ull;
                if (l < 4 * NB) {
                    const int w = l % NB, wi = w + (cut >> 6), sh = cut & 63;
                    const u64 lo_ = wi < NB ? pl[(l / NB) * NB + wi] : 0ull, hi_ = wi + 1 < NB ? pl[(l / NB) * NB + wi + 1] : 0ull;
                    v = sh ? (lo_ >> sh) | (hi_ << (64 - sh)) : lo_;
                }
                PG_SYNC();
                if (l < 4 * NB) pl[l] = v;
                PG_SYNC();
                len = len > cut ? len - cut : 0;
            }
        }
        S.len = len;
        S.M = max_mismatch_at(prm.mm_bp, len);
        S.T = S.M + S.add_mm + 1;
        S.thr = (int)uni((int)KA(B, thr_tab)[len]);
        const int J0 = pg_seed_depth(len, S.T, 0), J1 = pg_seed_depth(len, S.T, 1);
        const u32 b0 = (u32)min(S.T - 1, max_mismatch_at(prm.mm_bp, J0 < 0 ? 0 : J0) + S.add_mm),
                  b1 = (u32)min(S.T - 1, max_mismatch_at(prm.mm_bp, J1 < 0 ? 0 : J1) + S.add_mm);
        S.depth = (u32)(J0 < 0 ? 0 : J0) | ((u32)(J1 < 0 ? 0 : J1) << 8) | (b0 << 16) | (b1 << 24);
        S.jmask[0] = J0 > 1 ? (low32(J0) & ~1u) : 0u;
        S.jmask[1] = J1 > 1 ? (low32(J1) & ~1u) : 0u;
        S.ro = 0u;
        const u32 f0 = (u32)uni((int)(u32)(qplanes[QP_NN * NB] | qplanes[QP_OO * NB])) & 1u,
                  f1 = (u32)uni((int)(u32)(qplanes[4 * NB + QP_NN * NB] | qplanes[4 * NB + QP_OO * NB])) & 1u;
        flags &= ~(PG_RF_FIRST_OK_FWD | PG_RF_FIRST_OK_REV);
        if (!f0 && len > 0) flags |= PG_RF_FIRST_OK_FWD;
        if (!f1 && len > 0) flags |= PG_RF_FIRST_OK_REV;
    };
    if (EXACT) {
        auto lead = [&](const u64 *oo) {
            int n = 0;
            for (int w = 0; w < NB; w++) {
                const u64 x = (u64)(u32)uni((int)(u32)oo[w]) | ((u64)(u32)uni((int)(u32)(oo[w] >> 32)) << 32);
                if (x == ~0ull) { n += 64; continue; }
                n += __ffsll((long long)~x) - 1;
                break;
            }
            return n < len ? n : len;
        };
        ja = lead(qplanes + QP_OO * NB);
        jb = lead(qplanes + 4 * NB + QP_OO * NB);
        S.add_mm = PRM(add_mm, PG_DEF_ADD_MM);
    }
    const bool do_close = (mode & PG_MODE_CLOSE) != 0, do_far = (mode & PG_MODE_FAR) != 0;
    int flipped = 0, close_max = 0, n_close = 0;
    u32 close_last = 0, close_base = 0, alg = 0u;
    u32 unused0 = 0u, unused1 = 0u;
    u32 unused_valid = 0u;
    Acc<NB, Id> A;
    u32 fits = 1u;

    if (do_close) {
        int close_bases = 0;
        if (flags & PG_RF_CLOSE_OK) {
            const int w1s = (int)ra[0], isz = (int)ra[1];
            const u32 plus = flags & PG_RF_PLUS;
            S.bps = PRM(min_close, PG_DEF_MIN_CLOSE);
            S.sf = S.min_perfect >= S.bps ? 4u : (S.bps + 16 <= 32 ? 2u : 0u);
            const int w1e = w1s + 3 * isz;
            const u32 shared_grid = (flags / PG_RF_SHARED_GRID) & 1u;
            u32 cr0 = 0u, cr1 = 0u;
            u32 vr = 0u;
            u32 co0 = 0u, co1 = 0u;
            u32 vo = 0u;
            int ps = 0, pe = 0, nsurv_eval = 0;
            PG_STOP_AT(S, 11);
            auto attempt = [&](const int att, const bool plus_k, const bool staged = false) __attribute__((always_inline)) -> bool {
                const int Rg = att >> 1;
#ifdef PG_TIMING
                PG_T(S, S.t_base + 2);
                S.t_base = att == 0 ? 1 : 4;
#endif
                flipped = (att == 1 || att == 2) ? 1 : 0;
                if (EXACT && (att == 1 || att == 3)) {
                    ex_apply(att == 1 ? 1 : 2);
                    cr0 = cr1 = co0 = co1 = 0u;
                    vr = vo = 0u;
                }
                if (EXACT && len - 1 < PRM(min_close, PG_DEF_MIN_CLOSE)) return false;
                Query<NB> Q;
                Q.qp = qplanes + (!flipped ? 4 * NB : 0);
                Q.o1_ = !flipped;
                if (plus_k) {
                    Q.cF_ = !flipped; Q.cB_ = false; Q.allowF_ = true; Q.allowB_ = false;
                } else {
                    Q.cB_ = flipped; Q.cF_ = false; Q.allowF_ = false; Q.allowB_ = true;
                }
                const int s1 = Rg ? w1s : w1s + isz, e1 = Rg ? w1e : w1s + 2 * isz;
                Q.first_ok_ = (flags & (flipped ? PG_RF_FIRST_OK_FWD : PG_RF_FIRST_OK_REV)) != 0u;
                close_bases = e1 > s1 ? e1 - s1 : 0;
                if (att != 2) {
                    A.reset();
                    S.cap_state = 255;
                    S.nsurv = 0;
                    nsurv_eval = 0;
                    ps = pe = 0;
                }
                if (att == 1 || att == 3) {
                    const u32 t0 = cr0, t1 = cr1;
                    const u32 tv = vr;
                    cr0 = co0; cr1 = co1; vr = vo;
                    co0 = t0; co1 = t1; vo = tv;
                }
                const bool own_grid = att == 0 && !shared_grid;
                PG_STOP_AT_V(S, 12, true);
                if (staged)
                    scan_staged<NB, NS, Id, SM>(S, Q, A, own_grid ? s1 : w1s, s1, e1, w1s, PG_LANE, shared_grid, cr0, cr1, vr);
                else
                scan_range<NB, NS, Id, !DEF, SM>(ref, S, Q, A, chr_wo, own_grid ? s1 : w1s, s1, e1, own_grid ? e1 : w1e, ps, pe, w1s, 0u,
                                   PG_LANE, (att == 1 || att == 2 ? 1u : 0u) | shared_grid, cr0, cr1, vr);
                PG_STOPPED_V(S, true);
                PG_STOP_AT_V(S, 19, true);
                ps = s1;
                pe = e1;
                if (S.nsurv != nsurv_eval) {
                    nsurv_eval = S.nsurv;
                    Eval<NB, Id> E;
                    PG_DC(S, 0);
                    evaluate<NB, Id, SE>(S, A, E, PG_LANE);
                    PG_STOP_AT_V(S, 20, true);
                    close_max = uni(E.max_len);
                    if (uni(E.n_runs) > 0) {
                        u64 kept[NB];
                        n_close = uni(count_kept<NB, Id, SE>(E, true, kept));
                        if (n_close <= (int)PG_RES_CLOSE) {
                            close_base = res_base;
                            fits = res_fits;
                        } else
                            close_base = pool_alloc(B, n_close, lane, fits);
                        PG_DC(S, 20);
                        if (fits) emit_runs<NB, Id, SE>(S, true, false, chr, w1s, nullptr, E, kept, KA(B, pool) + close_base, PG_LANE);
                        const u64 idl = (u64)E.id_last;
                        const int pl = w1s + (int)(u32)(idl & ((1ull << IdFmt<Id>::RB) - 1ull));
                        close_last = ((idl >> IdFmt<Id>::RB) & 1ull) ? (u32)(pl - close_max + 1) : (u32)(pl + close_max - 1);
                        PG_STOP_AT_V(S, 21, true);
                        return true;
                    }
                }
                return false;
            };
            const bool staged0 = !EXACT && (int)ra[2] < (int)ra[3] && isz <= (int)PG_CHUNK && (flags & PG_RF_FIRST_OK_REV) != 0u;
            bool found = false;
            int att0 = 0;
            if (staged0) {
                found = plus ? attempt(0, true, true) : attempt(0, false, true);
                att0 = 1;
            }
            if (!found)
                for (int att = att0; att < 4; att++)
                    if (attempt(att, plus != 0u)) break;
            PG_STOPPED(S);
        }
        if (n_close == 0) { flipped = 0; close_max = 0; }
        if (EXACT) {
            if (n_close == 0) ex_stage = 2;
            flipped = ex_stage == 1 ? 1 : (ex_stage == 2 ? 2 : 0);
        }
        alg = (u32)(8 * len + 3 * (close_bases + 2 * len) + 96 * n_close);
    } else {
        const uint4 o1 = ((const uint4 *)record_ptr<5>(KA(B, out), rid))[1];
        close_last = (u32)uni((int)o1.x);
        close_max = uni((int)(o1.y & 0xffffu));
        flipped = uni((int)((o1.y >> 16) & 0xffu));
        alg = (u32)uni((int)o1.z) << 3;
        if (EXACT) ex_apply(flipped);
    }
    const int rc_out = flipped;
    if (EXACT || !do_close) flipped &= 1;

#ifdef PG_TIMING
    PG_T(S, S.t_base + 2);
    S.t_base = 7;
#endif
    PG_STOP_AT(S, 22);
    int n_far = 0, far_max = 0;
    u32 far_base = 0;
#if defined(PG_STOP) && PG_STOP == 2
    if (uni(opaque(1))) close_max = 0;
#endif
    if (do_far && close_max > 0 && len - 1 >= 10) {
        S.bps = 10;
        S.sf = S.min_perfect >= 10 ? 4u : 2u;
        Query<NB> Q;
        Q.qp = qplanes + (flipped ? 4 * NB : 0);
        Q.o1_ = flipped != 0;
        Q.cF_ = flipped; Q.cB_ = !flipped;
        Q.allowF_ = Q.allowB_ = true;
        Q.first_ok_ = (flags & (flipped ? PG_RF_FIRST_OK_REV : PG_RF_FIRST_OK_FWD)) != 0u;
        if (Q.first_ok_) {
            u32x4 rc;
            asm volatile("s_load_dwordx4 %0, %1, 0x30\n\ts_waitcnt lgkmcnt(0)" : "=&s"(rc) : "s"(record_ptr<7>(KA(B, in), rid)));
            const int chr_size = (int)rc[0];
            S.jmask[1] = LEN > 0 ? pg_fixed_len_row((uint32_t)LEN).jmask1 : rc[3];
            PG_STOP_AT(S, 35);
            int far_bases = 0;
            auto far_update = [&](int origin, const pg_window *bdw, int qmask) {
                Eval<NB, Id> E;
                PG_DC(S, 4);
                evaluate<NB, Id, SE>(S, A, E, PG_LANE, qmask);
                const int mx = uni(E.max_len);
                if (mx >= far_max) {
                    far_max = mx;
                    n_far = uni(E.n_runs);
                    far_base = 0;
                    if (n_far > 0) {
                        u64 kept[NB];
                        (void)count_kept<NB, Id, SE>(E, false, kept);
                        if (n_far <= (int)PG_RES_FAR) {
                            far_base = res_base + PG_RES_CLOSE;
                            fits &= res_fits;
                        } else {
                            u32 f2 = 1u;
                            far_base = pool_alloc(B, n_far, lane, f2);
                            fits &= f2;
                        }
                        PG_DC(S, 20);
                        if (fits) emit_runs<NB, Id, SE>(S, false, true, chr, origin, bdw, E, kept, KA(B, pool) + far_base, PG_LANE);
                    }
                }
            };
            bool done = false;
            const pg_window *bd_all = KA(B, bd);
            if (bd_all && rc[1] != 0u) {
                const int nbd = (int)rc[1];
                const pg_window *bd = bd_all + rc[2];
                A.reset();
                S.cap_state = 255;
                S.nsurv = 0;
                for (int w = 0; w < nbd; w++) {
                    const pg_window bw = bd[w];
                    const int st = bw.start < 0 ? bw.end - 1 : bw.start;
                    const bool own_chr = uni(bw.chr_id) == chr;
                    const int csz = own_chr ? chr_size : chr_size_of<NB>(ref, S, uni(bw.chr_id));
                    const int s = st < 0 ? 0 : st, e = bw.end > csz ? csz : bw.end;
                    far_bases += (e > s ? e - s : 0) + 2 * len;
                    scan_range<NB, NS, Id, !DEF, SM>(ref, S, Q, A, own_chr ? chr_wo : chr_word_off_of<NB>(ref, S, uni(bw.chr_id)), s, s, e, e, 0, 0, st,
                                       (u32)w, PG_LANE, false, unused0, unused1, unused_valid);
                    PG_STOPPED(S);
                }
                if (S.nsurv > 0) far_update(0, bd, 15);
                done = far_max + close_max >= len;
            }
            if (!done) {
                const int center = (int)close_last;
                const int k_mri = PRM(max_range_index, PG_DEF_MAX_RANGE_INDEX);
                const u32 k_spacer = PRM(spacer, PG_DEF_SPACER);
                const int maxspan = 64 << (2 * k_mri);
                const int origin = center - maxspan;
                const int g0 = center - (int)PG_CHUNK / 2;
                const u32 reach = (u32)maxspan + k_spacer;
                const bool noclip = reach >= k_spacer && (u32)center > reach && (u32)chr_size > reach && (u32)center < (u32)chr_size - reach;
                int emax;
                if (noclip || (u32)center + (u32)maxspan + k_spacer < (u32)chr_size) emax = center + maxspan;
                else emax = chr_size - (int)k_spacer;
                u32 cacheF = 0u, cacheB = 0u;
                u32 cache_valid = 0u;
                int ps = 0, pe = 0, nsurv_eval = 0;
                A.reset();
                S.cap_state = 255;
                if (k_mri >= 3) S.sf |= 1u;
                S.nsurv = 0;
                auto range_of = [&](int span, int &s, int &e) {
                    if ((u32)center > (u32)span + k_spacer) s = center - span; else s = (int)k_spacer;
                    if ((u32)center + (u32)span + k_spacer < (u32)chr_size) e = center + span;
                    else e = chr_size - (int)k_spacer;
                };
                int r_first = 0;
                PG_STOP_AT(S, 36);
                {
                    const int R = k_mri < 2 ? k_mri : 2;
                    int rs[3], re[3];
#pragma unroll
                    for (int r = 0; r < 3; r++) {
                        const int span = 64 << (2 * (r < R ? r : R));
                        if (noclip) { rs[r] = center - span; re[r] = center + span; }
                        else range_of(span, rs[r], re[r]);
                        rs[r] = uni(rs[r]);
                        re[r] = uni(re[r]);
                    }
                    PG_STOP_AT(S, 23);
                    if (rs[R] < re[R]) {
                        const int wb = g0 - 64 * NB;
                        const int se = emax < g0 + (int)PG_CHUNK ? emax : g0 + (int)PG_CHUNK;
                        if (!(chr_wo == S.win_wo && S.wbase == wb && se + 64 * NB <= S.win_hi))
                            stage_window<NB>(ref, S, chr_wo, wb, se + 64 * NB, lane);
                        PG_STOP_AT(S, 24);
                        u32 mF = 0u, mB = 0u;
                        seed_filter<NB, NS, true>(S, Q, false, false, lane, mF, mB);
                        PG_STOP_AT(S, 25);
                        cacheF = mF;
                        cacheB = mB;
                        cache_valid = 1u;
                        const int pbase = g0 + 32 * lane;
                        const u32 rmask = low32_lane(re[R] - pbase) & ~low32_lane(rs[R] - pbase);
                        mF &= rmask;
                        mB &= rmask;
                        const u32 cnt = (u32)(__popc(mF) + __popc(mB));
                        const u32 incl = wave_scan(cnt);
                        const int total = (int)read_lane(incl, 63);
                        PG_STOP_AT(S, 26);
                        if (total <= PG_PASS(NB)) {
                            r_first = R + 1;
                            ps = rs[R];
                            pe = re[R];
                            if (total > 0) {
                                int slot = (int)(incl - cnt);
                                PG_SYNC();
                                while (mF != 0u) {
                                    const int bit = __ffs((int)mF) - 1;
                                    mF &= mF - 1u;
                                    S.queue[slot] = (uint16_t)((u32)(64 * NB + 32 * lane + bit) << 1);
                                    slot++;
                                }
                                while (mB != 0u) {
                                    const int bit = __ffs((int)mB) - 1;
                                    mB &= mB - 1u;
                                    S.queue[slot] = (uint16_t)(((u32)(64 * NB + 32 * lane + bit) << 1) | 1u);
                                    slot++;
                                }
                                S.nsurv += total;
                                S.nsurv_total += (u32)total;
                                PG_SYNC();
                                PG_STOP_AT(S, 27);
                                int ring_n[3];
                                PG_T(S, 7);
                                fold_candidates<NB, Id, true, SM>(S, Q, A, wb, origin, 0u, total, lane,
                                                              Rings{ true, rs[0], re[0], rs[1], re[1] }, ring_n);
                                PG_STOPPED(S);
                                PG_STOP_AT(S, 30);
                                PG_T(S, 8);
                                for (int r = 0; r <= R; r++) {
                                    if (uni(ring_n[r]) > 0) {
                                        u64 longm[NB];
#pragma unroll
                                        for (int k = 0; k < NB; k++) longm[k] = read_lane(S.ringB[r * NB + k], 0);
                                        fold_tier_b<NB, Id, SM>(S, Q, A, longm, lane);
                                        far_update(origin, nullptr, r == 0 ? 1 : (r == 1 ? 3 : 15));
                                    }
                                    if (far_max + close_max >= len) {
                                        done = true;
                                        ps = rs[r];
                                        pe = re[r];
                                        break;
                                    }
                                }
                                nsurv_eval = S.nsurv;
                            }
                        }
                    }
                    PG_STOP_AT(S, 31);
                }
                int span = 64 << (2 * r_first);
                for (int r = r_first; r <= k_mri && !done; r++, span *= 4) {
                    int s, e;
                    range_of(span, s, e);
                    if (s < e) {
                        scan_range<NB, NS, Id, !DEF, SM>(ref, S, Q, A, chr_wo, g0, s, e, emax, ps, pe, origin, 0u, PG_LANE, true,
                                           cacheF, cacheB, cache_valid);
                        PG_STOPPED(S);
                        if (ps < pe) {
                            ps = s < ps ? s : ps;
                            pe = e > pe ? e : pe;
                        } else {
                            ps = s; pe = e;
                        }
                    }
                    if (S.nsurv != nsurv_eval) {
                        nsurv_eval = S.nsurv;
                        far_update(origin, nullptr, 15);
                    }
                    if (far_max + close_max >= len) break;
                }
                far_bases += (pe - ps) + 2 * len;
            }
            alg += (u32)(3 * far_bases + 96 * n_far);
        }
    }
    PG_STOP_AT(S, 32);
    PG_T(S, 9);
    alg = (alg + 4u) >> 3;
    if (PG_LANE == 0) {
        uint4 *op = (uint4 *)record_ptr<5>(KA(B, out), rid);
        if (do_close) {
            op[0] = make_uint4(close_base, (u32)n_close, far_base, (u32)n_far);
#ifdef PG_DIAG
            op[1] = make_uint4(close_last, (u32)close_max | ((u32)rc_out << 16), alg, S.dg);
#else
            op[1] = make_uint4(close_last, (u32)close_max | ((u32)rc_out << 16), alg, (u32)S.nsurv_total);
#endif
        } else {
            u32 *o = (u32 *)op;
            o[2] = far_base;
            o[3] = (u32)n_far;
            o[6] = alg;
            o[7] += (u32)S.nsurv_total;
        }
    }
}
#undef PG_LANE

template <int PB>
__device__ __forceinline__ void pack_block(const PgSoaIn &a, PgInRec *in, const u32 lo, const u32 r0, const u32 nb, const u32 lane);

template <int NB, int NS, typename Id, int mode, bool DEF>
__global__ __launch_bounds__(WAVE, PG_WAVES(NB, Id)) void pg_search_kernel(PgDevRef ref, PgDevParams prm,
                                                         PgDevBatch B, uint32_t max_len, uint32_t levels)
{
    constexpr int LEN = 0;
#include "pg_search_kernel_body.h"
}
template <int NB, int NS, int LEN>
__global__ __launch_bounds__(WAVE, PG_WAVES(NB, u32)) void pg_search_fixed_kernel(PgDevRef ref, PgDevParams prm,
                                                         PgDevBatch B, uint32_t max_len, uint32_t levels)
{
    static_assert(LEN > 64 * (NB - 1) && LEN <= 64 * NB, "the block class of the length");
    typedef u32 Id;
    constexpr int mode = PG_MODE_BOTH;
    constexpr bool DEF = true;
#include "pg_search_kernel_body.h"
}

template <int mode>
__global__ __launch_bounds__(WAVE, PG_WAVES(8, u64)) void pg_search_exact_kernel(PgDevRef ref, PgDevParams prm, PgDevBatch B,
                                                                               uint32_t max_len, uint32_t levels)
{
    constexpr int NB = 8;
    typedef u64 Id;
    __shared__ Lds<NB, Id> lds;
    const int lane = threadIdx.x;
    for (int L = lane; L < 64 * NB + 64; L += WAVE) lds.mm_tab[L] = (uint8_t)max_mismatch_at(prm.mm_bp, L);
    PG_SYNC();
    Search S;
    S.queue = lds.queue;
    S.win = lds.win;
    S.bufA = lds.bufA;
    S.bufB = lds.bufB;
    S.hdrB = lds.hdrB;
    S.ringB = lds.ringB;
    S.accB = lds.accB;
    S.mm_tab = lds.mm_tab;
    S.chr_tab = lds.chr_tab;
    u64 *qplanes = lds.qp;
    if (lane < 8 * NB) qplanes[lane] = 0ull;
#ifdef PG_TIMING
    S.t_acc = lds.t_acc;
    S.t_last = &lds.t_last;
    S.t_base = 1;
#endif
    const uint32_t n_list = *KA(B, exact_count), first = KA(B, first_read), n = KA(B, n_reads);
    const uint32_t *list = KA(B, exact_list);
    for (uint32_t i = blockIdx.x; i < n_list; i += gridDim.x) {
        const uint32_t rid = (u32)uni((int)list[i]);
        if (rid - first >= n) continue;
        u32 res = 0u;
        const u32 shard = blockIdx.x & (PG_POOL_SHARDS - 1u);
        uint32_t *cur = KA(B, pool_used) + shard * 16u;
        if (lane == 0) res = atomicAdd(cur, (u32)PG_RESERVE);
        res = (u32)uni((int)res);
        const u32 res_fits = (u64)res + (u64)PG_RESERVE <= (u64)KA(B, pool_shard_cap) ? 1u : 0u;
        res += shard * KA(B, pool_shard_cap);
        search_read<NB, 5, Id, mode, false, true>(ref, prm, B, S, qplanes, rid, 0, lane_now(), res, res_fits);
    }
}
extern "C" int pg_launch_search_exact(const PgDevRef *ref, const PgDevParams *prm, const PgDevBatch *batch, int mode,
                                      uint32_t max_len, uint32_t levels, void *stream, PgLaunchRec *rec)
{
    if (rec) *rec = PgLaunchRec{};
    if (batch->n_reads == 0 || !batch->exact_list) return 0;
    if (rec) *rec = PgLaunchRec{PG_KERNEL_EXACT, 0, 0, 0, mode == PG_MODE_BOTH || mode == PG_MODE_CLOSE ? mode : PG_MODE_FAR, 0, 0};
    hipStream_t st = (hipStream_t)stream;
    const dim3 grid(64), block(WAVE);
    if (mode == PG_MODE_BOTH)
        hipLaunchKernelGGL((pg_search_exact_kernel<PG_MODE_BOTH>), grid, block, 0, st, *ref, *prm, *batch, max_len, levels);
    else if (mode == PG_MODE_CLOSE)
        hipLaunchKernelGGL((pg_search_exact_kernel<PG_MODE_CLOSE>), grid, block, 0, st, *ref, *prm, *batch, max_len, levels);
    else
        hipLaunchKernelGGL((pg_search_exact_kernel<PG_MODE_FAR>), grid, block, 0, st, *ref, *prm, *batch, max_len, levels);
    return (int)hipGetLastError();
}

static_assert(offsetof(PgKArgs, ref) == 0 && offsetof(PgKArgs, prm) == sizeof(PgDevRef) && alignof(PgDevRef) == 8 && alignof(PgDevParams) == 4 &&
              offsetof(PgKArgs, B) == ((sizeof(PgDevRef) + sizeof(PgDevParams) + 7) & ~(size_t)7) &&
              offsetof(PgKArgs, max_len) == offsetof(PgKArgs, B) + sizeof(PgDevBatch) && offsetof(PgKArgs, levels) == offsetof(PgKArgs, max_len) + 4,
              "PgKArgs mirrors the kernarg segment of pg_search_kernel(PgDevRef, PgDevParams, PgDevBatch, uint32_t, uint32_t)");
__global__ void pg_kargs_check_kernel(PgDevRef ref, PgDevParams prm, PgDevBatch B, uint32_t max_len, uint32_t levels)
{
    u32 bad = 0u;
#define PG_CHK(obj, m) bad += (u64)KA(obj, m) != (u64)obj.m ? 1u : 0u
    PG_CHK(ref, lo); PG_CHK(ref, hi); PG_CHK(ref, nn); PG_CHK(ref, chr_word_off); PG_CHK(ref, chr_size); PG_CHK(ref, n_chr);
    PG_CHK(prm, max_range_index); PG_CHK(prm, add_mm); PG_CHK(prm, min_perfect); PG_CHK(prm, min_close); PG_CHK(prm, spacer);
    PG_CHK(B, n_reads); PG_CHK(B, first_read); PG_CHK(B, in); PG_CHK(B, out); PG_CHK(B, seq); PG_CHK(B, planes); PG_CHK(B, plane_blocks);
    PG_CHK(B, bd); PG_CHK(B, pool); PG_CHK(B, pool_shard_cap); PG_CHK(B, pool_used); PG_CHK(B, work_ctr); PG_CHK(B, claim);
    PG_CHK(B, exact_list); PG_CHK(B, exact_count); PG_CHK(B, thr_tab); PG_CHK(B, soa);
#undef PG_CHK
    {
        const u32 *glo, *ghi, *gnn;
        karg_load3<(int)offsetof(PgKArgs, ref.lo)>(glo, ghi, gnn);
        bad += (glo != ref.lo ? 1u : 0u) + (ghi != ref.hi ? 1u : 0u) + (gnn != ref.nn ? 1u : 0u);
    }
    bad += karg_load<uint32_t>((int)offsetof(PgKArgs, max_len)) != max_len ? 1u : 0u;
    bad += karg_load<uint32_t>((int)offsetof(PgKArgs, levels)) != levels ? 1u : 0u;
    if (threadIdx.x == 0) *B.work_ctr = bad;
}
extern "C" int pg_debug_kargs_check(const PgDevRef *ref, const PgDevParams *prm, const PgDevBatch *batch, uint32_t max_len, uint32_t levels,
                                    uint32_t *scratch_dev, void *stream)
{
    PgDevBatch b = *batch;
    b.work_ctr = scratch_dev;
    hipStream_t st = (hipStream_t)stream;
    hipLaunchKernelGGL(pg_kargs_check_kernel, dim3(1), dim3(WAVE), 0, st, *ref, *prm, b, max_len, levels);
    uint32_t bad = ~0u;
    if (hipMemcpyAsync(&bad, scratch_dev, sizeof bad, hipMemcpyDeviceToHost, st) != hipSuccess || hipStreamSynchronize(st) != hipSuccess) return -1;
    return (int)bad;
}

template <int NB, int NS, typename Id, bool DEF>
static void note_search(PgLaunchRec *rec, int *n_rec, int mode, const PgDevBatch *batch)
{
    if (rec && *n_rec < PG_LAUNCH_RECS_MAX)
        rec[(*n_rec)++] = PgLaunchRec{PG_KERNEL_SEARCH, NB, NS, (int32_t)(8 * sizeof(Id)), mode, DEF ? 1 : 0, batch->soa ? 1 : 0};
}

template <int NB, int NS, typename Id, bool DEF>
static void launch_modes(const PgDevRef *ref, const PgDevParams *prm, const PgDevBatch *batch, int mode,
                         uint32_t max_len, uint32_t levels, hipStream_t st, unsigned lds_pad, dim3 grid, dim3 block,
                         PgLaunchRec *rec, int *n_rec)
{
    const bool fused = !pg_env_switches()->split_launch;
    if (mode == PG_MODE_BOTH && fused) {
        hipLaunchKernelGGL((pg_search_kernel<NB, NS, Id, PG_MODE_BOTH, DEF>), grid, block, lds_pad, st,
                           *ref, *prm, *batch, max_len, levels);
        note_search<NB, NS, Id, DEF>(rec, n_rec, PG_MODE_BOTH, batch);
        return;
    }
#ifdef PG_ONLY_BENCH
    abort();
#else
    if (mode & PG_MODE_CLOSE) {
        hipLaunchKernelGGL((pg_search_kernel<NB, NS, Id, PG_MODE_CLOSE, DEF>), grid, block, lds_pad, st,
                           *ref, *prm, *batch, max_len, levels);
        note_search<NB, NS, Id, DEF>(rec, n_rec, PG_MODE_CLOSE, batch);
    }
    if (mode & PG_MODE_FAR) {
        if (mode & PG_MODE_CLOSE) (void)hipMemsetAsync(batch->work_ctr, 0, PG_N_XCD * 16u * sizeof(uint32_t), st);
        hipLaunchKernelGGL((pg_search_kernel<NB, NS, Id, PG_MODE_FAR, DEF>), grid, block, lds_pad, st,
                           *ref, *prm, *batch, max_len, levels);
        note_search<NB, NS, Id, DEF>(rec, n_rec, PG_MODE_FAR, batch);
    }
#endif
}

template <int NB, int NS>
static bool launch_fixed(const PgDevRef *ref, const PgDevParams *prm, const PgDevBatch *batch, uint32_t max_len, uint32_t levels,
                         hipStream_t st, unsigned lds_pad, dim3 grid, dim3 block, uint32_t len)
{
    if (len == 0u || len != max_len || levels != pg_fixed_len_row(len).lvl >> 24) return false;
#define PG_FIXED(nb, ns, L)                                                                                                           \
    if constexpr (NB == nb && NS == ns)                                                                                               \
        if (len == L) {                                                                                                               \
            hipLaunchKernelGGL((pg_search_fixed_kernel<nb, ns, L>), grid, block, lds_pad, st, *ref, *prm, *batch, max_len, levels);   \
            return true;                                                                                                              \
        }
    PG_FIXED(2, 3, 100)
    PG_FIXED(2, 3, 101)
    PG_FIXED(3, 3, 150)
    PG_FIXED(3, 3, 151)
#undef PG_FIXED
    return false;
}

template <int NB, int NS, typename Id>
static void launch_ns(const PgDevRef *ref, const PgDevParams *prm, const PgDevBatch *batch, int mode,
                   uint32_t max_len, uint32_t levels, hipStream_t st, unsigned lds_pad, PgLaunchRec *rec, int *n_rec,
                   uint32_t uniform_len, uint32_t *fixed_len)
{
    static int n_cu = 0;
    if (!n_cu) {
        int dev = 0;
        hipDeviceProp_t p;
        if (hipGetDevice(&dev) == hipSuccess && hipGetDeviceProperties(&p, dev) == hipSuccess) n_cu = p.multiProcessorCount;
        if (n_cu <= 0) n_cu = 256;
    }
    const uint32_t chunks = (batch->n_reads + PG_CLAIM - 1) / PG_CLAIM + PG_N_XCD;
    const uint32_t want = (uint32_t)n_cu * 4u * (uint32_t)PG_WAVES(NB, Id);
    dim3 grid(chunks < want ? chunks : want), block(WAVE);
    PgDevBatch with_claim = *batch;
    {
        const uint32_t per_wg = (batch->n_reads + grid.x - 1u) / grid.x, n_claims = (per_wg + PG_CLAIM - 1u) / PG_CLAIM;
        with_claim.claim = per_wg >= 8u * PG_CLAIM ? PG_CLAIM : (per_wg + n_claims - 1u) / n_claims;
        if (with_claim.claim == 0u) with_claim.claim = 1u;
        if (batch->soa) {
            const uint32_t dflt = prm->max_range_index <= 2 && per_wg >= 32u * PG_PACK_CLAIM_LONG ? PG_PACK_CLAIM_LONG : PG_PACK_CLAIM;
            const uint32_t pc = pg_env_switches()->pack_claim ? pg_env_switches()->pack_claim : dflt;
            with_claim.claim = pc > 64u ? 64u : pc;
        }
    }
    batch = &with_claim;
    if (PG_WIN_DYN_BYTES(NB) != 0u && prm->max_range_index >= 3) lds_pad += PG_WIN_DYN_BYTES(NB);
    constexpr bool HAS_DEF = NS <= 4 && sizeof(Id) == 4;
    const bool def = HAS_DEF && !pg_env_switches()->generic_kernels && prm->max_range_index == PG_DEF_MAX_RANGE_INDEX &&
                     prm->add_mm == PG_DEF_ADD_MM && prm->min_perfect == PG_DEF_MIN_PERFECT && prm->min_close == PG_DEF_MIN_CLOSE &&
                     prm->spacer == PG_DEF_SPACER;
    if constexpr (HAS_DEF) {
        if (def) {
            if (mode == PG_MODE_BOTH && !pg_env_switches()->split_launch && !pg_env_switches()->no_fixed_len &&
                launch_fixed<NB, NS>(ref, prm, batch, max_len, levels, st, lds_pad, grid, block, uniform_len)) {
                note_search<NB, NS, Id, true>(rec, n_rec, PG_MODE_BOTH, batch);
                *fixed_len = uniform_len;
                return;
            }
            launch_modes<NB, NS, Id, true>(ref, prm, batch, mode, max_len, levels, st, lds_pad, grid, block, rec, n_rec);
            return;
        }
    }
    launch_modes<NB, NS, Id, false>(ref, prm, batch, mode, max_len, levels, st, lds_pad, grid, block, rec, n_rec);
}

template <int NB, typename Id>
static void launch(const PgDevRef *ref, const PgDevParams *prm, const PgDevBatch *batch, int mode,
                   uint32_t max_len, uint32_t levels, hipStream_t st, unsigned lds_pad, PgLaunchRec *rec, int *n_rec,
                   uint32_t uniform_len, uint32_t *fixed_len)
{
    if (levels <= 8) launch_ns<NB, 3, Id>(ref, prm, batch, mode, max_len, levels, st, lds_pad, rec, n_rec, uniform_len, fixed_len);
#ifdef PG_ONLY_BENCH
    else abort();
#else
    else if (levels <= 16) launch_ns<NB, 4, Id>(ref, prm, batch, mode, max_len, levels, st, lds_pad, rec, n_rec, uniform_len, fixed_len);
    else launch_ns<NB, 5, Id>(ref, prm, batch, mode, max_len, levels, st, lds_pad, rec, n_rec, uniform_len, fixed_len);
#endif
}

#define PG_PACK_UNROLL 2
#define PG_PACK_GRID 65536u
static_assert(sizeof(PgOutRec) == 32, "record_ptr<5>");
static_assert(sizeof(PgInRec) == 128 && offsetof(PgInRec, prog) == 64 && offsetof(PgInRec, w1s) == 0 && offsetof(PgInRec, isz) == 4 && offsetof(PgInRec, stage_s) == 8 &&
              offsetof(PgInRec, stage_e) == 12 && offsetof(PgInRec, chr_wo_lo) == 16 && offsetof(PgInRec, lenf) == 24 && offsetof(PgInRec, lvl) == 28 &&
              offsetof(PgInRec, depth) == 32 && offsetof(PgInRec, jmask0) == 36 && offsetof(PgInRec, ro) == 40 && offsetof(PgInRec, chr) == 44 &&
              offsetof(PgInRec, chr_size) == 48 && offsetof(PgInRec, bd_cnt) == 52 && offsetof(PgInRec, bd_off) == 56 && offsetof(PgInRec, jmask1) == 60,
              "pg_pack_kernel writes PgInRec as four uint4; search_read reads it as dwords 0..7, 8..11, 12..15");
struct PgDw3 { u32 x, y, z; };
template <int PB>
__device__ __forceinline__ void pack_block(const PgSoaIn &a, PgInRec *in, const u32 lo, const u32 r0, const u32 nb, const u32 lane)
{
    constexpr u32 LPR = 8u * PB;
    constexpr u32 RPW = 64u / LPR;
    constexpr u32 STEPS = (64u + RPW - 1u) / RPW;
    constexpr u32 U = PG_PACK_UNROLL < STEPS ? PG_PACK_UNROLL : STEPS;
    static_assert(STEPS % U == 0, "unroll must divide the steps");
    const u32 slot = lane / LPR, L = lane % LPR;
    const u32 D = L >> 2, pl = L & 3u, idx0 = 8u * L;
    {
        u32 so_lo = 0u, so_hi = 0u, len = 0u;
        if (lane < nb) {
            const u32 ii = lo + r0 + lane;
            uint4 o;
            __builtin_memcpy(&o, __builtin_assume_aligned(a.seq_off + ii, 8), 16);
            so_lo = o.x;
            so_hi = o.y;
            len = o.z - o.x;
            const u32 lc = len < 512u ? len : 511u;
            const int isz = (int)a.isz[ii];
            const int apos = a.pos[ii] + (int32_t)a.spacer;
            const u32 strand = a.strand[ii];
            const int chr = a.chr[ii];
            const u64 wo = a.chr_word_off[chr];
            uint4 lt0, lt1;
            __builtin_memcpy(&lt0, __builtin_assume_aligned(a.len_tab + lc, 16), 16);
            __builtin_memcpy(&lt1, __builtin_assume_aligned((const char *)(a.len_tab + lc) + 16, 16), 16);
            u32 flags = 0u;
            const bool plus = strand == (u32)'+';
            if ((int)len - 1 >= a.min_close && (plus || strand == (u32)'-')) flags |= PG_RF_CLOSE_OK;
            if (plus) flags |= PG_RF_PLUS;
            const bool shared = isz > 0 && 3 * isz <= (int)PG_CHUNK;
            if (shared) flags |= PG_RF_SHARED_GRID;
            if (len) {
                const u64 at = (u64)so_lo | ((u64)so_hi << 32);
                const u32 c0 = a.seq[at], c1 = a.seq[at + len - 1u];
                if (c0 == 'A' || c0 == 'C' || c0 == 'G' || c0 == 'T') flags |= PG_RF_FIRST_OK_FWD;
                if (c1 == 'A' || c1 == 'C' || c1 == 'G' || c1 == 'T') flags |= PG_RF_FIRST_OK_REV;
            }
            const int w1s = plus ? apos - isz : apos - 2 * isz;
            int ss = 0, se = 0;
            if (flags & PG_RF_CLOSE_OK) {
                const int s1 = shared ? w1s : w1s + isz, e1 = shared ? w1s + 3 * isz : w1s + 2 * isz;
                if (s1 < e1) {
                    ss = s1;
                    se = e1 < s1 + (int)PG_CHUNK ? e1 : s1 + (int)PG_CHUNK;
                }
            }
            uint4 q0, q1, q2, q3;
            q0.x = (u32)w1s;
            q0.y = (u32)isz;
            q0.z = (u32)ss;
            q0.w = (u32)se;
            q1.x = (u32)wo;
            q1.y = (u32)(wo >> 32);
            q1.z = (len & 0xffffu) | (flags << 16);
            q1.w = lt0.x;
            q2.x = lt0.y;
            q2.y = lt0.z;
            q2.z = lt0.w;
            q2.w = (u32)chr;
            q3.x = a.chr_size[chr];
            q3.y = q3.z = 0u;
            q3.w = lt1.x;
            if (a.bd_off) {
                uint4 w;
                __builtin_memcpy(&w, __builtin_assume_aligned(a.bd_off + ii, 8), 16);
                q3.z = w.x;
                q3.y = w.z - w.x;
            }
            uint4 *dst = (uint4 *)(in + ii);
            dst[0] = q0;
            dst[1] = q1;
            dst[2] = q2;
            dst[3] = q3;
        }
        for (u32 s = 0; s < STEPS && s * RPW < nb; s += U) {
            u32 d0[U], d1[U], d2[U], ln[U], sh[U];
            bool act[U];
#pragma unroll
            for (u32 u = 0; u < U; u++) {
                const u32 src = (s + u) * RPW + slot;
                act[u] = slot < RPW && src < nb;
                const u32 olo = (u32)__shfl((int)so_lo, (int)(src & 63u)), ohi = (u32)__shfl((int)so_hi, (int)(src & 63u));
                ln[u] = (u32)__shfl((int)len, (int)(src & 63u));
                if (!act[u]) ln[u] = 0u;
                const u64 A = ((u64)olo | ((u64)ohi << 32)) + idx0;
                sh[u] = (u32)A & 3u;
                d0[u] = d1[u] = d2[u] = 0u;
                if (idx0 < ln[u]) {
                    PgDw3 t;
                    __builtin_memcpy(&t, __builtin_assume_aligned((const u32 *)a.seq + (A >> 2), 4), 12);
                    d0[u] = t.x;
                    d1[u] = t.y;
                    d2[u] = t.z;
                }
            }
#pragma unroll
            for (u32 u = 0; u < U; u++) {
                const u32 w0 = __builtin_amdgcn_alignbyte(d1[u], d0[u], sh[u]), w1 = __builtin_amdgcn_alignbyte(d2[u], d1[u], sh[u]);
                const u32 nv = ln[u] > idx0 ? (ln[u] - idx0 < 8u ? ln[u] - idx0 : 8u) : 0u;
                const u32 vm0 = nv >= 4u ? 0x80808080u : (0x80808080u & ((1u << (8u * nv)) - 1u));
                const u32 vm1 = nv >= 8u ? 0x80808080u : (nv > 4u ? (0x80808080u & ((1u << (8u * (nv - 4u))) - 1u)) : 0u);
                u32 P;
                {
                    auto nibbles = [](u32 w, u32 vm) {
                        const u32 code = (w >> 1) & 0x03030303u;
                        const u32 x = w ^ __builtin_amdgcn_perm(0x47544341u, 0x47544341u, code);
                        const u32 V = ~((((x & 0x7f7f7f7fu) + 0x7f7f7f7fu) | x)) & vm;
                        const u32 xn = w ^ 0x4e4e4e4eu;
                        const u32 N = ~((((xn & 0x7f7f7f7fu) + 0x7f7f7f7fu) | xn)) & vm;
                        const u32 O = vm & ~(V | N);
                        const u32 c = code & ((V >> 7) | (V >> 6));
                        return ((c ^ (c >> 1)) & 0x01010101u) | (c & 0x02020202u) | (N >> 5) | (O >> 4);
                    };
                    u32 Z = nibbles(w0, vm0) | (nibbles(w1, vm1) << 4);
                    u32 t;
                    t = (Z ^ (Z >> 7)) & 0x884422u;  Z ^= t | (t << 7);
                    t = (Z ^ (Z >> 14)) & 0x8844u;   Z ^= t | (t << 14);
                    t = (Z ^ (Z >> 21)) & 0x88u;     Z ^= t | (t << 21);
                    P = Z;
                }
                const u32 t = (u32)__shfl_xor((int)P, 2);
                const u32 y = (L & 2u) ? ((t >> 16) | (P & 0xffff0000u)) : ((P & 0xffffu) | (t << 16));
                const u32 x = (u32)__shfl_xor((int)y, 1);
                const u32 Fd = (L & 1u) ? (((x >> 8) & 0x00ff00ffu) | (y & 0xff00ff00u)) : ((y & 0x00ff00ffu) | ((x & 0x00ff00ffu) << 8));
                const int q = (int)ln[u] - 32 - 32 * (int)D;
                const int dF = q >> 5;
                const u32 sb = (u32)q & 31u;
                const int j0 = dF < 0 ? 0 : (dF >= 2 * PB ? 2 * PB - 1 : dF), j1 = dF + 1 < 0 ? 0 : (dF + 1 >= 2 * PB ? 2 * PB - 1 : dF + 1);
                u32 fl = (u32)__shfl((int)Fd, (int)((slot * LPR + 4u * (u32)j0 + pl) & 63u));
                u32 fh = (u32)__shfl((int)Fd, (int)((slot * LPR + 4u * (u32)j1 + pl) & 63u));
                if (dF < 0 || dF >= 2 * PB) fl = 0u;
                if (dF + 1 < 0 || dF + 1 >= 2 * PB) fh = 0u;
                const u32 Rd = __brev(__builtin_amdgcn_alignbit(fh, fl, sb));
                if (act[u]) {
                    u32 *dst = (u32 *)a.planes + (size_t)(lo + r0 + (s + u) * RPW + slot) * (16u * PB);
                    dst[2u * PB * pl + D] = Fd;
                    dst[2u * PB * (4u + pl) + D] = Rd;
                }
                {
                    const u32 q0 = slot * LPR;
                    const u32 flo = (u32)__shfl((int)Fd, (int)(q0 & 63u)), fhi = (u32)__shfl((int)Fd, (int)((q0 + 1u) & 63u)),
                              fnn = (u32)__shfl((int)Fd, (int)((q0 + 2u) & 63u));
                    const u32 rlo = (u32)__shfl((int)Rd, (int)(q0 & 63u)), rhi = (u32)__shfl((int)Rd, (int)((q0 + 1u) & 63u)),
                              rnn = (u32)__shfl((int)Rd, (int)((q0 + 2u) & 63u));
                    u32 *rec = (u32 *)(in + (lo + r0 + (s + u) * RPW + slot));
#pragma unroll
                    for (u32 h = 0; h < (LPR >= 16u ? 1u : 2u); h++) {
                        const u32 q = L + 8u * h;
                        if (act[u] && q < 16u) {
                            const u32 g = q & 7u;
                            const bool o1 = q >= 8u;
                            const u32 plo = o1 ? rlo : flo, phi = o1 ? rhi : fhi, pnn = o1 ? rnn : fnn;
                            const u32 j = 3u * g + 1u;
                            const u32 l3 = (((plo >> j) & 7u) * 0x4081u) & 0x010101u, h3 = (((phi >> j) & 7u) * 0x4081u) & 0x010101u,
                                      n3 = (((pnn >> j) & 7u) * 0x4081u) & 0x010101u;
                            u32 w = l3 | (h3 << 1);
                            if (o1) w ^= 0x030303u;
                            w = (w & ~(n3 * 3u)) | (n3 << 2);
                            w |= 0x30303030u;
                            if (g == 0u) {
                                u32 x = (plo & 1u) | ((phi & 1u) << 1);
                                if (o1) x ^= 3u;
                                if (pnn & 1u) x = 4u;
                                w |= x << 24;
                            }
                            rec[16u + q] = w;
                        }
                    }
                    if (act[u] && L == 3u && ((Fd | Rd) & 0x1ffffffu)) atomicAnd(rec + 10, ~PG_RO_OK);
                    if (act[u] && pl == 3u && Fd != 0u && a.exact_list) {
                        const u32 old = atomicOr(rec + 6, (u32)PG_RF_EXACT << 16);
                        if (!(old & ((u32)PG_RF_EXACT << 16))) a.exact_list[atomicAdd(a.exact_count, 1u)] = lo + r0 + (s + u) * RPW + slot;
                    }
                }
            }
        }
    }
}
template <int PB>
__global__ __launch_bounds__(256) void pg_pack_kernel(PgSoaIn a, PgInRec *in, uint32_t lo, uint32_t cnt)
{
    const u32 n_blocks = (cnt + 63u) >> 6, n_waves = gridDim.x * 4u;
    for (u32 g = blockIdx.x * 4u + (threadIdx.x >> 6); g < n_blocks; g += n_waves) {
        const u32 r0 = g << 6;
        pack_block<PB>(a, in, lo, r0, cnt - r0 < 64u ? cnt - r0 : 64u, threadIdx.x & 63u);
    }
}

__global__ void pg_pack_close_kernel(PgSoaOut a, PgOutRec *out, uint32_t n)
{
    const uint32_t i = blockIdx.x * blockDim.x + threadIdx.x;
    if (i >= n) return;
    PgOutRec r;
    r.close_off = r.close_cnt = r.far_off = r.far_cnt = 0;
    r.close_last = a.close_last[i];
    r.close_max = a.close_max[i];
    r.rc_flag = a.rc_flag[i];
    r.pad = 0;
    r.alg = 0;
    r.reserved = 0;
    out[i] = r;
}

template <int PB>
static void launch_pack(const PgSoaIn *soa, PgInRec *in, uint32_t lo, uint32_t cnt, hipStream_t st)
{
    const uint32_t want = (cnt + 255u) / 256u, cap = PG_PACK_GRID;
    pg_pack_kernel<PB><<<want < cap ? want : cap, 256, 0, st>>>(*soa, in, lo, cnt);
}
extern "C" int pg_pack_reads(const PgSoaIn *soa, PgInRec *in, uint32_t lo, uint32_t cnt, void *stream, PgLaunchRec *rec)
{
    if (rec) *rec = PgLaunchRec{};
    if (cnt) {
        if (rec) *rec = PgLaunchRec{PG_KERNEL_PACK, (int32_t)soa->plane_blocks, 0, 0, 0, 0, 0};
        hipStream_t st = (hipStream_t)stream;
        switch (soa->plane_blocks) {
        case 1: launch_pack<1>(soa, in, lo, cnt, st); break;
        case 2: launch_pack<2>(soa, in, lo, cnt, st); break;
        case 3: launch_pack<3>(soa, in, lo, cnt, st); break;
        case 4: launch_pack<4>(soa, in, lo, cnt, st); break;
        case 8: launch_pack<8>(soa, in, lo, cnt, st); break;
        default: return (int)hipErrorInvalidValue;
        }
    }
    return (int)hipGetLastError();
}

extern "C" int pg_pack_close_summary(const PgSoaOut *soa, PgOutRec *out, uint32_t n, void *stream)
{
    if (n) pg_pack_close_kernel<<<(n + 255u) / 256u, 256, 0, (hipStream_t)stream>>>(*soa, out, n);
    return (int)hipGetLastError();
}

__global__ void pg_calib_stream(const u32 *src, size_t n, u32 *sink)
{
    u32 acc = 0;
    for (size_t i = (size_t)blockIdx.x * blockDim.x + threadIdx.x; i < n; i += (size_t)gridDim.x * blockDim.x)
        acc ^= src[i];
    if (acc == 0x12345678u) *sink = acc;
}

extern "C" int pg_debug_calib_stream(const void *src, size_t n_dwords, void *sink)
{
    hipLaunchKernelGGL(pg_calib_stream, dim3(4096), dim3(256), 0, 0, (const u32 *)src, n_dwords, (u32 *)sink);
    return (int)hipDeviceSynchronize();
}

extern "C" int pg_debug_occupancy(uint32_t max_len, uint32_t levels, int small_ids, int *close_blocks,
                                  int *far_blocks, unsigned *lds_bytes)
{
    (void)max_len;
    (void)levels;
    *lds_bytes = (unsigned)sizeof(Lds<2, u32>);
    hipError_t e1, e2;
#ifdef PG_ONLY_BENCH
    (void)small_ids;
    e1 = e2 = hipOccupancyMaxActiveBlocksPerMultiprocessor(far_blocks, pg_search_kernel<2, 3, u32, PG_MODE_BOTH, false>, WAVE, 0);
    *close_blocks = *far_blocks;
    return (int)e1;
#endif
    if (small_ids) {
        e1 = hipOccupancyMaxActiveBlocksPerMultiprocessor(close_blocks, pg_search_kernel<2, 3, u32, PG_MODE_CLOSE, false>, WAVE, 0);
        e2 = hipOccupancyMaxActiveBlocksPerMultiprocessor(far_blocks, pg_search_kernel<2, 3, u32, PG_MODE_BOTH, false>, WAVE, 0);
    } else {
        e1 = hipOccupancyMaxActiveBlocksPerMultiprocessor(close_blocks, pg_search_kernel<2, 3, u64, PG_MODE_CLOSE, false>, WAVE, 0);
        e2 = hipOccupancyMaxActiveBlocksPerMultiprocessor(far_blocks, pg_search_kernel<2, 3, u64, PG_MODE_BOTH, false>, WAVE, 0);
    }
    return (int)e1 | (int)e2;
}

static int search_class_blocks(uint32_t max_len, int small_ids)
{
    const int nb = max_len <= 128 ? 2 : (max_len <= 256 ? 4 : 8);
    if (!small_ids) return nb;
    return max_len <= 64 ? 1 : (nb == 2 ? 2 : (max_len <= 192 ? 3 : nb));
}
extern "C" int pg_pack_in_place_ok(int mode, uint32_t max_len, int small_ids, uint32_t n_reads, uint32_t plane_blocks)
{
    if ((mode == PG_MODE_BOTH && pg_env_switches()->split_launch) || pg_env_switches()->no_pack_in_place) return 0;
    if (mode != PG_MODE_BOTH && mode != PG_MODE_CLOSE && mode != PG_MODE_FAR) return 0;
    if ((uint32_t)search_class_blocks(max_len, small_ids) != plane_blocks) return 0;
    return n_reads >= pg_env_switches()->pack_in_place_min ? 1 : 0;
}

extern "C" int pg_launch_search(const PgDevRef *ref, const PgDevParams *prm, const PgDevBatch *batch,
                                int mode, uint32_t max_len, uint32_t levels, int small_ids, void *stream,
                                PgLaunchRec *rec, int *n_rec, uint32_t uniform_len, uint32_t *fixed_len)
{
    int n_local = 0;
    uint32_t fixed_local = 0;
    if (!n_rec) n_rec = &n_local;
    if (!fixed_len) fixed_len = &fixed_local;
    *n_rec = 0;
    *fixed_len = 0;
    if (batch->n_reads == 0) return 0;
    if (batch->soa && !pg_pack_in_place_ok(mode, max_len, small_ids, batch->n_reads, batch->plane_blocks)) return (int)hipErrorInvalidValue;
    hipStream_t st = (hipStream_t)stream;
    const unsigned lds_pad = pg_env_switches()->lds_pad;
    const int nb = max_len <= 128 ? 2 : (max_len <= 256 ? 4 : 8);
#ifdef PG_ONLY_BENCH
    if (!small_ids || max_len > 192) abort();
    if (nb == 2 && max_len > 64) launch<2, u32>(ref, prm, batch, mode, max_len, levels, st, lds_pad, rec, n_rec, uniform_len, fixed_len);
    else launch<3, u32>(ref, prm, batch, mode, max_len, levels, st, lds_pad, rec, n_rec, uniform_len, fixed_len);
    return (int)hipGetLastError();
#else
    if (small_ids) {
        if (max_len <= 64) launch<1, u32>(ref, prm, batch, mode, max_len, levels, st, lds_pad, rec, n_rec, uniform_len, fixed_len);
        else if (nb == 2) launch<2, u32>(ref, prm, batch, mode, max_len, levels, st, lds_pad, rec, n_rec, uniform_len, fixed_len);
        else if (max_len <= 192) launch<3, u32>(ref, prm, batch, mode, max_len, levels, st, lds_pad, rec, n_rec, uniform_len, fixed_len);
        else if (nb == 4) launch<4, u32>(ref, prm, batch, mode, max_len, levels, st, lds_pad, rec, n_rec, uniform_len, fixed_len);
        else launch<8, u32>(ref, prm, batch, mode, max_len, levels, st, lds_pad, rec, n_rec, uniform_len, fixed_len);
    } else {
        if (nb == 2) launch<2, u64>(ref, prm, batch, mode, max_len, levels, st, lds_pad, rec, n_rec, uniform_len, fixed_len);
        else if (nb == 4) launch<4, u64>(ref, prm, batch, mode, max_len, levels, st, lds_pad, rec, n_rec, uniform_len, fixed_len);
        else launch<8, u64>(ref, prm, batch, mode, max_len, levels, st, lds_pad, rec, n_rec, uniform_len, fixed_len);
    }
    return (int)hipGetLastError();
#endif
}

#include <hipcub/block/block_scan.hpp>
#include <hipcub/block/block_reduce.hpp>

__global__ __launch_bounds__(256) void pg_deliver_scan1(const PgOutRec *out, uint32_t cnt, uint8_t *rc_flag, uint32_t *close_last,
                                                        uint16_t *close_max, uint2 *local, uint2 *blk)
{
    typedef hipcub::BlockScan<uint32_t, 256> Scan;
    __shared__ typename Scan::TempStorage tc, tf;
    const uint32_t i = blockIdx.x * 256u + threadIdx.x;
    uint32_t c = 0, f = 0;
    if (i < cnt) {
        const PgOutRec r = out[i];
        rc_flag[i] = r.rc_flag;
        close_last[i] = r.close_last;
        close_max[i] = r.close_max;
        c = r.close_cnt;
        f = r.far_cnt;
    }
    uint32_t ec, ef, sc, sf;
    Scan(tc).ExclusiveSum(c, ec, sc);
    Scan(tf).ExclusiveSum(f, ef, sf);
    if (i < cnt) local[i] = make_uint2(ec, ef);
    if (threadIdx.x == 0) blk[blockIdx.x] = make_uint2(sc, sf);
}

__global__ __launch_bounds__(1024) void pg_deliver_scan2(uint2 *blk, uint32_t nblk, unsigned long long *run_tot, unsigned long long *info,
                                                         const uint32_t *pool_used)
{
    typedef hipcub::BlockScan<uint32_t, 1024> Scan;
    typedef hipcub::BlockReduce<uint32_t, 1024> Reduce;
    __shared__ typename Scan::TempStorage tc, tf;
    __shared__ typename Reduce::TempStorage tr;
    const uint32_t worst = Reduce(tr).Reduce(threadIdx.x < PG_POOL_SHARDS ? pool_used[threadIdx.x * 16u] : 0u, hipcub::Max());
    uint2 v[4];
    uint32_t tx = 0u, ty = 0u;
#pragma unroll
    for (int j = 0; j < 4; j++) {
        const uint32_t idx = threadIdx.x * 4u + (uint32_t)j;
        v[j] = idx < nblk ? blk[idx] : make_uint2(0u, 0u);
        tx += v[j].x;
        ty += v[j].y;
    }
    uint32_t ec, ef, sc, sf;
    Scan(tc).ExclusiveSum(tx, ec, sc);
    Scan(tf).ExclusiveSum(ty, ef, sf);
#pragma unroll
    for (int j = 0; j < 4; j++) {
        const uint32_t idx = threadIdx.x * 4u + (uint32_t)j;
        if (idx < nblk) blk[idx] = make_uint2(ec, ef);
        ec += v[j].x;
        ef += v[j].y;
    }
    if (threadIdx.x == 0) {
        info[0] = run_tot[0];
        info[1] = run_tot[1];
        info[2] = sc;
        info[3] = sf;
        info[4] = worst;
        info[5] = 0ull;
        run_tot[0] += sc;
        run_tot[1] += sf;
    }
}

__global__ __launch_bounds__(256) void pg_deliver_gather(const PgOutRec *out, uint32_t cnt, const uint2 *local, const uint2 *blk,
                                                         const unsigned long long *info, const pg_run *pool, unsigned long long pool_runs,
                                                         pg_run *close_runs, pg_run *far_runs, unsigned long long cap,
                                                         unsigned long long *close_off, unsigned long long *far_off,
                                                         unsigned long long *overflow)
{
    const uint32_t i = blockIdx.x * 256u + threadIdx.x;
    if (i >= cnt) return;
    const PgOutRec r = out[i];
    const uint2 l = local[i], b = blk[blockIdx.x];
    const unsigned long long oc = info[0] + b.x + l.x, of = info[1] + b.y + l.y;
    close_off[i] = oc;
    far_off[i] = of;
    if (!far_runs) {
        if (info[2] + info[3] > cap) {
            *overflow = 1ull;
            return;
        }
        far_runs = close_runs + info[2];
    } else if (oc + r.close_cnt > cap || of + r.far_cnt > cap) {
        *overflow = 1ull;
        return;
    }
    if ((unsigned long long)r.close_off + r.close_cnt > pool_runs || (unsigned long long)r.far_off + r.far_cnt > pool_runs) {
        *overflow = 1ull;
        return;
    }
    const u32 *sc = (const u32 *)(pool + r.close_off), *sf = (const u32 *)(pool + r.far_off);
    u32 *dc = (u32 *)(close_runs + oc), *df = (u32 *)(far_runs + of);
    for (uint32_t k = 0; k < 3u * r.close_cnt; k++) dc[k] = sc[k];
    for (uint32_t k = 0; k < 3u * r.far_cnt; k++) df[k] = sf[k];
}

extern "C" int pg_deliver_scan(const PgOutRec *out, uint32_t cnt, uint8_t *rc_flag, uint32_t *close_last, uint16_t *close_max,
                               void *local, void *blk, unsigned long long *run_tot, unsigned long long *info,
                               const uint32_t *pool_used, void *stream)
{
    if (!cnt || cnt > PG_DELIVER_CHUNK) return cnt ? (int)hipErrorInvalidValue : 0;
    hipStream_t st = (hipStream_t)stream;
    const uint32_t nblk = (cnt + 255u) / 256u;
    pg_deliver_scan1<<<nblk, 256, 0, st>>>(out, cnt, rc_flag, close_last, close_max, (uint2 *)local, (uint2 *)blk);
    pg_deliver_scan2<<<1, 1024, 0, st>>>((uint2 *)blk, nblk, run_tot, info, pool_used);
    return (int)hipGetLastError();
}

extern "C" int pg_deliver_gather_runs(const PgOutRec *out, uint32_t cnt, const void *local, const void *blk, unsigned long long *info,
                                      const pg_run *pool, unsigned long long pool_runs, pg_run *close_runs, pg_run *far_runs,
                                      unsigned long long cap, unsigned long long *close_off, unsigned long long *far_off, void *stream)
{
    if (!cnt || cnt > PG_DELIVER_CHUNK) return cnt ? (int)hipErrorInvalidValue : 0;
    pg_deliver_gather<<<(cnt + 255u) / 256u, 256, 0, (hipStream_t)stream>>>(out, cnt, (const uint2 *)local, (const uint2 *)blk, info, pool,
                                                                            pool_runs, close_runs, far_runs, cap, close_off, far_off, info + 5);
    return (int)hipGetLastError();
}

extern "C" int pg_deliver_chunk(const PgOutRec *out, uint32_t cnt, uint8_t *rc_flag, uint32_t *close_last, uint16_t *close_max,
                                void *local, void *blk, unsigned long long *run_tot, unsigned long long *info,
                                const pg_run *pool, unsigned long long pool_runs, pg_run *close_runs, pg_run *far_runs,
                                unsigned long long cap, unsigned long long *close_off, unsigned long long *far_off,
                                const uint32_t *pool_used, void *stream)
{
    if (int rc = pg_deliver_scan(out, cnt, rc_flag, close_last, close_max, local, blk, run_tot, info, pool_used, stream)) return rc;
    return pg_deliver_gather_runs(out, cnt, local, blk, info, pool, pool_runs, close_runs, far_runs, cap, close_off, far_off, stream);
}
```

Before: 550.3 million reads/s.

## Add short-form fold step with inverted verdict encoding and unclamped tier-A loop

Introduces a short-form fold step (SF), enabled for default parameters with 32-bit ids on selected kernel instantiations. It precomputes the candidate verdict at enqueue time: the hamming-ok flag is folded into the stored word so the tier-A and tier-B checks become a single AND or OR, and the accumulator uses an inverted ok convention (0 = passed). The tier-A loop drops the per-iteration index clamp and, in the non-mixed path, also the bounds test, using byte offsets into LDS. A static assert checks that any address this can form stays inside the static LDS. The aim is fewer ALU ops per folded candidate, at the cost of more template instantiations and a subtle encoding invariant that every consumer must respect.

```diff
diff --git a/pindel_amd/csrc/pg_fold_step.h b/pindel_amd/csrc/pg_fold_step.h
--- /dev/null
+++ b/pindel_amd/csrc/pg_fold_step.h
@@ -0,0 +1,87 @@
+#ifndef PG_FOLD_STEP_H
+#define PG_FOLD_STEP_H
+#include <stdint.h>
+
+#if defined(__HIPCC__)
+#define PG_FS_FN __host__ __device__ __forceinline__
+#else
+#define PG_FS_FN static inline
+#endif
+
+#define PG_FS_BIG 0xffffu
+
+PG_FS_FN uint32_t pg_fs_med3(uint32_t a, uint32_t b, uint32_t c)
+{
+#if defined(__HIP_DEVICE_COMPILE__)
+    uint32_t r;
+    asm("v_med3_u32 %0, %1, %2, %3" : "=v"(r) : "v"(a), "v"(b), "v"(c));
+    return r;
+#else
+    const uint32_t lo = a < b ? a : b, hi = a < b ? b : a;
+    return c < lo ? lo : (c > hi ? hi : c);
+#endif
+}
+
+template <bool SF> PG_FS_FN uint32_t pg_fs_none() { return SF ? 1u : 0u; }
+template <bool SF> PG_FS_FN bool pg_fs_passed(uint32_t v) { return SF ? v == 0u : v != 0u; }
+
+constexpr bool pg_fs_window_never_empty(int bps, int min_perfect) { return min_perfect >= 1 && min_perfect <= bps; }
+
+template <typename Id>
+PG_FS_FN void pg_fs_fold(uint32_t &m1, uint32_t &m2, Id &id, uint32_t &v, uint32_t k, Id cid, uint32_t vc)
+{
+    const bool lt = k < m1;
+    m2 = pg_fs_med3(m1, m2, k);
+    id = lt ? cid : id;
+    v = lt ? vc : v;
+    m1 = k < m1 ? k : m1;
+}
+template <typename Id>
+PG_FS_FN void pg_fs_merge(uint32_t &a1, uint32_t &a2, Id &aid, uint32_t &av, uint32_t b1, uint32_t b2, Id bid, uint32_t bv)
+{
+    const bool lt = b1 < a1;
+    const uint32_t hi1 = a1 > b1 ? a1 : b1, lo2 = a2 < b2 ? a2 : b2;
+    a2 = hi1 < lo2 ? hi1 : lo2;
+    aid = lt ? bid : aid;
+    av = lt ? bv : av;
+    a1 = lt ? b1 : a1;
+}
+
+template <bool SF> PG_FS_FN uint32_t pg_fs_entry_a_y(uint32_t sne, uint32_t hamok)
+{
+    return SF ? (hamok ? sne : ~0u) : sne;
+}
+template <bool SF> PG_FS_FN uint32_t pg_fs_entry_a_w(uint32_t meta) { return SF ? 0u : meta; }
+template <bool SF> PG_FS_FN uint32_t pg_fs_verdict_a(uint32_t ey, uint32_t ew, uint32_t bpm)
+{
+    return SF ? (ey & bpm) : ((ey & bpm) == 0u ? (ew >> 31) : 0u);
+}
+PG_FS_FN uint32_t pg_fs_level_a(uint32_t ex, uint32_t mk)
+{
+#if defined(__HIP_DEVICE_COMPILE__)
+    return (uint32_t)__popc(ex & mk);
+#else
+    return (uint32_t)__builtin_popcount(ex & mk);
+#endif
+}
+
+template <bool SF> PG_FS_FN uint32_t pg_fs_hdr_b_y(uint32_t meta, uint32_t hamok)
+{
+    return SF ? (hamok ? 0u : ~0u) : meta;
+}
+template <bool SF> PG_FS_FN uint32_t pg_fs_verdict_b(uint64_t bad, uint32_t hy)
+{
+    return SF ? ((uint32_t)bad | (uint32_t)(bad >> 32) | hy) : (bad == 0ull ? (hy >> 31) : 0u);
+}
+
+template <bool SF> PG_FS_FN uint32_t pg_fs_accb_pack(uint32_t m1, uint32_t m2, uint32_t v)
+{
+    const uint32_t c2 = m2 < 0x7fffu ? m2 : 0x7fffu;
+    return m1 | (c2 << 16) | ((SF ? (v != 0u ? 1u : 0u) : v) << 31);
+}
+PG_FS_FN void pg_fs_accb_unpack(uint32_t x, uint32_t &m1, uint32_t &m2, uint32_t &v)
+{
+    m1 = x & 0xffffu; m2 = (x >> 16) & 0x7fffu; v = x >> 31;
+}
+
+#endif
diff --git a/pindel_amd/csrc/pg_kernels.hip b/pindel_amd/csrc/pg_kernels.hip
--- a/pindel_amd/csrc/pg_kernels.hip
+++ b/pindel_amd/csrc/pg_kernels.hip
@@ -5,6 +5,7 @@
 #include "pg_device.h"
 #include "pg_lane_masks.h"
 #include "pg_eval_masks.h"
+#include "pg_fold_step.h"
 
 typedef unsigned long long u64;
 typedef unsigned int u32;
@@ -146,6 +147,16 @@
     if (!DEF || EXACT) return false;
     if (LEN > 0) return true;
     return (NB == 3 && mode == PG_MODE_FAR) || (NB == 4 && NS == 4 && mode == PG_MODE_BOTH) || (NB == 8 && mode == PG_MODE_CLOSE);
+}
+template <int NB, int NS, typename Id, int mode, bool DEF, bool EXACT, int LEN>
+constexpr bool pg_short_fold()
+{
+    if (!pg_short_masks<NB, NS, mode, DEF, EXACT, LEN>() || sizeof(Id) != 4) return false;
+    if (LEN > 0) return true;
+    if (NB == 2 && NS == 3 && mode == PG_MODE_FAR) return false;
+    if (NB == 4 && (mode == PG_MODE_BOTH || mode == PG_MODE_CLOSE)) return false;
+    if (NB == 8 && NS == 4 && (mode == PG_MODE_CLOSE || mode == PG_MODE_FAR)) return false;
+    return true;
 }
 __device__ __forceinline__ int count_below(u64 m)
 {
@@ -214,12 +225,13 @@
     static __device__ __forceinline__ void load(const void *base, int i, u32 &m1, u32 &m2, u32 &ok, u32 &id)
     {
         const uint2 st = ((const uint2 *)base)[i];
-        m1 = st.x & 0xffffu; m2 = (st.x >> 16) & 0x7fffu; ok = st.x >> 31; id = st.y;
-    }
+        pg_fs_accb_unpack(st.x, m1, m2, ok);
+        id = st.y;
+    }
+    template <bool SF>
     static __device__ __forceinline__ void store(void *base, int i, u32 m1, u32 m2, u32 ok, u32 id)
     {
-        const u32 c2 = m2 < 0x7fffu ? m2 : 0x7fffu;
-        ((uint2 *)base)[i] = make_uint2(m1 | (c2 << 16) | (ok << 31), id);
+        ((uint2 *)base)[i] = make_uint2(pg_fs_accb_pack<SF>(m1, m2, ok), id);
     }
 };
 template <> struct AccB<u64> {
@@ -229,8 +241,10 @@
         const uint4 st = ((const uint4 *)base)[i];
         m1 = st.x; m2 = st.y & 0xffffu; ok = st.y >> 16; id = (u64)st.z | ((u64)st.w << 32);
     }
+    template <bool SF>
     static __device__ __forceinline__ void store(void *base, int i, u32 m1, u32 m2, u32 ok, u64 id)
     {
+        static_assert(!SF, "the short form of the fold step has 32-bit ids");
         ((uint4 *)base)[i] = make_uint4(m1, m2 | (ok << 16), (u32)id, (u32)(id >> 32));
     }
 };
@@ -298,18 +312,26 @@
 #ifdef PG_DIAG
     u32 dg;
 #endif
-#if defined(PG_DIAG) && PG_DIAG == 2
+#if defined(PG_DIAG) && PG_DIAG == 3
+#define PG_DG(S, sh) ((void)0)
+#define PG_DC(S, sh) ((void)0)
+#define PG_DC_IF(S, cond, sh) ((void)0)
+#define PG_DN(S, sh, n) (const_cast<Search &>(S).dg += (u32)(n) << (sh))
+#elif defined(PG_DIAG) && PG_DIAG == 2
 #define PG_DG(S, sh) ((void)0)
 #define PG_DC(S, sh) ((S).dg += 1u << (sh))
 #define PG_DC_IF(S, cond, sh) ((S).dg += (cond) ? 1u << (sh) : 0u)
+#define PG_DN(S, sh, n) ((void)0)
 #elif defined(PG_DIAG)
 #define PG_DG(S, sh) ((S).dg += 1u << (sh))
 #define PG_DC(S, sh) ((void)0)
 #define PG_DC_IF(S, cond, sh) ((void)0)
+#define PG_DN(S, sh, n) ((void)0)
 #else
 #define PG_DG(S, sh) ((void)0)
 #define PG_DC(S, sh) ((void)0)
 #define PG_DC_IF(S, cond, sh) ((void)0)
+#define PG_DN(S, sh, n) ((void)0)
 #endif
     int cap_state;
     u32 sf;
@@ -325,32 +347,25 @@
     u32 a1, a2, aok;
     Id aid;
     u32 dirty;
+    template <bool SF>
     __device__ __forceinline__ void reset()
     {
-        m1 = m2 = PG_BIG; ok = 0u; id = 0;
-        a1 = a2 = PG_BIG; aok = 0u; aid = 0;
+        m1 = m2 = PG_BIG; ok = pg_fs_none<SF>(); id = 0;
+        a1 = a2 = PG_BIG; aok = pg_fs_none<SF>(); aid = 0;
         dirty = 0u;
     }
 };
+static_assert(PG_FS_BIG == PG_BIG, "pg_fold_step.h: the level of no candidate");
 
 template <typename Id>
 __device__ __forceinline__ void fold(u32 &m1, u32 &m2, Id &id, u32 &ok, u32 k, Id cid, u32 okc)
 {
-    const bool lt = k < m1;
-    m2 = med3(m1, m2, k);
-    id = lt ? cid : id;
-    ok = lt ? okc : ok;
-    m1 = k < m1 ? k : m1;
+    pg_fs_fold<Id>(m1, m2, id, ok, k, cid, okc);
 }
 template <typename Id>
 __device__ __forceinline__ void merge(u32 &a1, u32 &a2, Id &aid, u32 &aok, u32 b1, u32 b2, Id bid, u32 bok)
 {
-    const bool lt = b1 < a1;
-    const u32 hi1 = a1 > b1 ? a1 : b1, lo2 = a2 < b2 ? a2 : b2;
-    a2 = hi1 < lo2 ? hi1 : lo2;
-    aid = lt ? bid : aid;
-    aok = lt ? bok : aok;
-    a1 = lt ? b1 : a1;
+    pg_fs_merge<Id>(a1, a2, aid, aok, b1, b2, bid, bok);
 }
 
 __device__ __forceinline__ int max_mismatch_at(const u32 *mm_bp, int L)
@@ -425,7 +440,7 @@
     int s0, e0, s1, e1;
 };
 
-template <int NB, typename Id, bool SM>
+template <int NB, typename Id, bool SM, bool SF>
 __device__ __forceinline__ void fold_tier_b(const Search &S, const Query<NB> &Q, Acc<NB, Id> &A, const u64 *longm, int lane)
 {
     constexpr int EW = NB;
@@ -452,6 +467,7 @@
         u64 mask = longm[r];
         if (mask == 0ull) continue;
         const int L = L0 + lB;
+        PG_DN(S, r == 0 ? 16 : 22, __popcll(mask));
         u64 Mk[NB], BP[NB], QN[NB];
 #pragma unroll
         for (int b = 0; b < NB; b++) {
@@ -462,7 +478,7 @@
         u32 m1 = A.m1, m2 = A.m2, ok = A.ok;
         Id wid = A.id;
         if (r > 0) {
-            m1 = m2 = PG_BIG; ok = 0u; wid = 0;
+            m1 = m2 = PG_BIG; ok = pg_fs_none<SF>(); wid = 0;
             if ((A.dirty >> r) & 1u) {
                 AccB<Id>::load(S.accB, (r - 1) * 64 + lB, m1, m2, ok, wid);
             }
@@ -482,20 +498,21 @@
                 k += (u32)__popcll(b < r ? m : (m & Mk[b]));
                 if (b + 1 >= r) bad |= (m ^ QN[b]) & BP[b];
             }
-            u32 okc = bad == 0ull ? (h.y >> 31) : 0u;
-            if (S.len_check()) okc = (u32)L >= ((h.y >> 24) & 0x7fu) ? okc : 0u;
+            u32 okc = pg_fs_verdict_b<SF>(bad, h.y);
+            if (!SF && S.len_check()) okc = (u32)L >= ((h.y >> 24) & 0x7fu) ? okc : 0u;
             const Id cid = sizeof(Id) == 8 ? (Id)((u64)h.x | ((u64)(h.y & 0xffffffu) << 32)) : (Id)h.x;
             fold<Id>(m1, m2, wid, ok, k, cid, okc);
         }
         if (r == 0) { A.m1 = m1; A.m2 = m2; A.ok = ok; A.id = wid; }
         else {
-            AccB<Id>::store(S.accB, (r - 1) * 64 + lB, m1, m2, ok, wid);
+            AccB<Id>::template store<SF>(S.accB, (r - 1) * 64 + lB, m1, m2, ok, wid);
+            PG_DN(S, 27, 1);
             A.dirty |= 1u << r;
         }
     }
 }
 
-template <int NB, typename Id, bool MIXED, bool SM>
+template <int NB, typename Id, bool MIXED, bool SM, bool SF>
 __device__ __forceinline__ void fold_candidates(const Search &S, const Query<NB> &Q, Acc<NB, Id> &A, int wbase,
                                                 int origin, u32 region, int n, int lane, const Rings &R, int *ring_n)
 {
@@ -572,7 +589,7 @@
             if (sht) {
                 const u64 mine = ring == 0 ? sh0 : (ring == 1 ? sh1 : sh2);
                 const int rank = count_below(mine) + (ring == 0 ? 0 : (ring == 1 ? n0 : n0 + n1));
-                S.bufA[rank] = make_uint4(m0lo, s0lo, (u32)id, meta);
+                S.bufA[rank] = make_uint4(m0lo, pg_fs_entry_a_y<SF>(s0lo, hamok), (u32)id, pg_fs_entry_a_w<SF>(meta));
             }
             qb = qd == 0 ? 0 : (qd == 1 ? n0 : n0 + n1 + (qd - 2));
             qs = qd < 2 ? 1 : 2;
@@ -594,7 +611,7 @@
         } else {
             if (sht) {
                 const int rank = count_below(shortm);
-                S.bufA[rank] = make_uint4(m0lo, s0lo, (u32)id, meta);
+                S.bufA[rank] = make_uint4(m0lo, pg_fs_entry_a_y<SF>(s0lo, hamok), (u32)id, pg_fs_entry_a_w<SF>(meta));
             }
             qb = qd;
             qs = 4;
@@ -605,10 +622,12 @@
             for (int r = 1; r < NB; r++) longm[r] = lngm & ballot64(kk[r] < S.T);
         }
     }
-    if (lng) S.hdrB[lane] = make_uint2((u32)id, meta);
+    if (lng) S.hdrB[lane] = make_uint2((u32)id, pg_fs_hdr_b_y<SF>(meta, hamok));
     PG_STOP_AT(const_cast<Search &>(S), (MIXED && R.on) ? 28 : 17);
     PG_SYNC();
     if (nA > 0) {
+        if (MIXED && R.on) PG_DN(S, 10, n_iter);
+        else { PG_DN(S, 0, nA >> 2); PG_DN(S, 6, (nA & 3) ? 1 : 0); }
         const int lA = opaque(lane);
         u32 mk, bpm;
         if (SM) {
@@ -619,17 +638,39 @@
             mk = low32_lane(L);
             bpm = mk & ~low32_lane(L - S.min_perfect);
         }
+        if constexpr (SF) {
+            typedef Lds<NB, Id> LdsT;
+            static_assert(offsetof(LdsT, bufA) == 0 && 16 * 3 * PG_PASS(NB) <= sizeof(LdsT) && PG_PASS(NB) <= 64,
+                          "tier A without the clamp: every index a quarter can form lies inside the static LDS");
+            const char *const listA = (const char *)S.bufA;
+            u32 at = 16u * (u32)qb;
+            const u32 end = 16u * (u32)qe;
+            auto step = [&](bool test) {
+                const uint4 e = *(const uint4 *)__builtin_assume_aligned(listA + at, 16);
+                u32 k = pg_fs_level_a(e.x, mk);
+                if (test) k = at < end ? k : PG_BIG;
+                fold<Id>(A.a1, A.a2, A.aid, A.aok, k, (Id)e.z, pg_fs_verdict_a<true>(e.y, e.w, bpm));
+            };
+            if (MIXED && R.on) {
+                for (int it = 0; it < n_iter; it++, at += 16u * (u32)qs) step(true);
+            } else {
+                const int n_full = nA >> 2;
+                for (int it = 0; it < n_full; it++, at += 64u) step(false);
+                if (nA & 3) step(true);
+            }
+        } else {
         int idx = qb;
         for (int it = 0; it < n_iter; it++, idx += qs) {
             const uint4 e = S.bufA[idx < 67 ? idx : 67];
             u32 k = (u32)__popc(e.x & mk);
             k = idx < qe ? k : PG_BIG;
-            const u32 okc = (e.y & bpm) == 0u ? (e.w >> 31) : 0u;
+            const u32 okc = pg_fs_verdict_a<false>(e.y, e.w, bpm);
             const Id cid = sizeof(Id) == 8 ? (Id)((u64)e.z | ((u64)(e.w & 0xffffffu) << 32)) : (Id)e.z;
             fold<Id>(A.a1, A.a2, A.aid, A.aok, k, cid, okc);
         }
-    }
-    if (!(MIXED && R.on)) fold_tier_b<NB, Id, SM>(S, Q, A, longm, lane);
+        }
+    }
+    if (!(MIXED && R.on)) fold_tier_b<NB, Id, SM, SF>(S, Q, A, longm, lane);
     PG_SYNC();
     PG_STOP_AT(const_cast<Search &>(S), (MIXED && R.on) ? 29 : 18);
 }
@@ -1094,7 +1135,7 @@
     seed_filter_run<NB, NS, DUAL>(S, Q, kindB, lane, jmask, g0mask, cap0, mF, mB);
 }
 
-template <int NB, int NS, typename Id, bool MIXED, bool W3, bool SM>
+template <int NB, int NS, typename Id, bool MIXED, bool W3, bool SM, bool SF>
 __device__ __forceinline__ void scan_impl(const PgDevRef &ref, Search &S,
                                           const Query<NB> &Q, Acc<NB, Id> &A, long long wo, int g0, int s, int e,
                                           int e_max, int xs, int xe, int origin, u32 region, int lane,
@@ -1163,7 +1204,7 @@
                 S.nsurv_total += (u32)n;
                 PG_SYNC();
                 PG_T(S, S.t_base);
-                fold_candidates<NB, Id, MIXED, SM>(S, Q, A, wb, origin, region, n, lane, Rings{ false, 0, 0, 0, 0 }, nullptr);
+                fold_candidates<NB, Id, MIXED, SM, SF>(S, Q, A, wb, origin, region, n, lane, Rings{ false, 0, 0, 0, 0 }, nullptr);
                 PG_STOPPED(S);
                 PG_T(S, S.t_base + 1);
                 slot -= n;
@@ -1227,14 +1268,14 @@
             PG_SYNC();
             PG_T(S, S.t_base);
             PG_STOP_AT(S, 16);
-            fold_candidates<NB, Id, MIXED, SM>(S, Q, A, wb, origin, region, n, lane, Rings{ false, 0, 0, 0, 0 }, nullptr);
+            fold_candidates<NB, Id, MIXED, SM, SF>(S, Q, A, wb, origin, region, n, lane, Rings{ false, 0, 0, 0, 0 }, nullptr);
             PG_STOPPED(S);
             PG_T(S, S.t_base + 1);
         }
     }
 }
 
-template <int NB, int NS, typename Id, bool W3, bool SM>
+template <int NB, int NS, typename Id, bool W3, bool SM, bool SF>
 __device__ __forceinline__ void scan_range(const PgDevRef &ref, Search &S,
                                            const Query<NB> &Q, Acc<NB, Id> &A, long long wo, int g0, int s, int e,
                                            int e_max, int xs, int xe, int origin, u32 region, int lane,
@@ -1242,14 +1283,14 @@
 {
     g0 = uni(g0); s = uni(s); e = uni(e); e_max = uni(e_max); xs = uni(xs); xe = uni(xe); origin = uni(origin);
     if (Q.allowF() && Q.allowB())
-        scan_impl<NB, NS, Id, true, W3, SM>(ref, S, Q, A, wo, g0, s, e, e_max, xs, xe, origin, region, lane,
+        scan_impl<NB, NS, Id, true, W3, SM, SF>(ref, S, Q, A, wo, g0, s, e, e_max, xs, xe, origin, region, lane,
                                     use_cache, cacheF, cacheB, cache_valid);
     else
-        scan_impl<NB, NS, Id, false, false, SM>(ref, S, Q, A, wo, g0, s, e, e_max, xs, xe, origin, region, lane,
+        scan_impl<NB, NS, Id, false, false, SM, SF>(ref, S, Q, A, wo, g0, s, e, e_max, xs, xe, origin, region, lane,
                                         use_cache, cacheF, cacheB, cache_valid);
 }
 
-template <int NB, int NS, typename Id, bool SM>
+template <int NB, int NS, typename Id, bool SM, bool SF>
 __device__ __forceinline__ void scan_staged(Search &S, const Query<NB> &Q, Acc<NB, Id> &A, int g0, int s, int e, int origin,
                                             int lane, u32 keep, u32 &cacheF, u32 &cacheB, u32 &cache_valid)
 {
@@ -1286,7 +1327,7 @@
         PG_SYNC();
         PG_T(S, S.t_base);
         PG_STOP_AT(S, 16);
-        fold_candidates<NB, Id, false, SM>(S, Q, A, wb, origin, 0u, n, lane, Rings{ false, 0, 0, 0, 0 }, nullptr);
+        fold_candidates<NB, Id, false, SM, SF>(S, Q, A, wb, origin, 0u, n, lane, Rings{ false, 0, 0, 0, 0 }, nullptr);
         PG_STOPPED(S);
         PG_T(S, S.t_base + 1);
     }
@@ -1314,7 +1355,7 @@
     return S.mm_tab[L];
 }
 
-template <int NB, typename Id, bool SE>
+template <int NB, typename Id, bool SE, bool SF>
 __device__ __forceinline__ void evaluate(Search &S, const Acc<NB, Id> &A, Eval<NB, Id> &E, int lane, int qmask = 15)
 {
     static_assert(PG_MM_BREAKS < 64, "the short form's reach rule: no level of a point reaches 64");
@@ -1326,12 +1367,13 @@
     u32 t1 = A.m1, t2 = A.m2, tok = A.ok;
     Id tid = A.id;
     if (S.tierA()) {
-        u32 a1 = PG_BIG, a2 = PG_BIG, aok = 0u;
+        u32 a1 = PG_BIG, a2 = PG_BIG, aok = pg_fs_none<SF>();
         Id aid = 0;
         if (lane < 16) { a1 = A.a1; a2 = A.a2; aok = A.aok; aid = A.aid; }
         if (qmask != 1) {
             PG_DC(S, 24);
-            S.bufA[lane] = make_uint4(A.a1, A.a2 | (A.aok << 16), (u32)A.aid, (u32)((u64)A.aid >> 32));
+            if (SF) S.bufA[lane] = make_uint4(A.a1, A.a2, (u32)A.aid, A.aok);
+            else S.bufA[lane] = make_uint4(A.a1, A.a2 | (A.aok << 16), (u32)A.aid, (u32)((u64)A.aid >> 32));
             PG_SYNC();
             if (lane < 16) {
 #pragma unroll
@@ -1339,7 +1381,8 @@
                     if (!((qmask >> q) & 1)) continue;
                     const uint4 o = S.bufA[lane + 16 * q];
                     const Id oid = sizeof(Id) == 8 ? (Id)((u64)o.z | ((u64)o.w << 32)) : (Id)o.z;
-                    merge<Id>(a1, a2, aid, aok, o.x, o.y & 0xffffu, oid, o.y >> 16);
+                    if (SF) merge<Id>(a1, a2, aid, aok, o.x, o.y, oid, o.w);
+                    else merge<Id>(a1, a2, aid, aok, o.x, o.y & 0xffffu, oid, o.y >> 16);
                 }
             }
             PG_SYNC();
@@ -1374,7 +1417,7 @@
         u32 m1 = t1, m2 = t2, ok = tok, mmL = mm0;
         Id wid = tid;
         if (r > 0) {
-            m1 = m2 = PG_BIG; ok = 0u; wid = 0;
+            m1 = m2 = PG_BIG; ok = pg_fs_none<SF>(); wid = 0;
             mmL = mm_of<NB>(S, L);
             if ((A.dirty >> r) & 1u) {
                 AccB<Id>::load(S.accB, (r - 1) * 64 + lane, m1, m2, ok, wid);
@@ -1385,11 +1428,11 @@
         const u64 ab = vm & ballot64(lo > mmL);
         u64 cm;
         if (SE) {
-            cm = vm & (~ab & (ab - 1ull)) & ballot64(m2 > m1 + (u32)S.add_mm) & ballot64(ok != 0u);
+            cm = vm & (~ab & (ab - 1ull)) & ballot64(m2 > m1 + (u32)S.add_mm) & (SF ? ballot64(ok == 0u) : ballot64(ok != 0u));
             if (pg_em_reach_needs_compare(r)) cm &= ballot64((u32)lane >= m1);
         } else
             cm = vm & (~ab & (ab - 1ull)) & ballot64(m1 <= (u32)S.M) & ballot64(m2 > m1 + (u32)S.add_mm) &
-                 ballot64((u32)L >= (u32)S.bps + m1) & ballot64(ok != 0u);
+                 ballot64((u32)L >= (u32)S.bps + m1) & (SF ? ballot64(ok == 0u) : ballot64(ok != 0u));
         PG_DC(S, 12);
         PG_DC_IF(S, cm == 0ull, 16);
         if (SE && cm == 0ull) {
@@ -1526,6 +1569,10 @@
     static_assert(PG_DEF_MIN_PERFECT <= PG_DEF_MIN_CLOSE && PG_DEF_MIN_PERFECT <= 10, "the short masks need min_perfect <= bps at both ends");
     constexpr bool SM = pg_short_masks<NB, NS, mode, DEF, EXACT, LEN>();
     constexpr bool SE = pg_short_eval<NB, NS, Id, mode, DEF, EXACT, LEN>();
+    constexpr bool SF = pg_short_fold<NB, NS, Id, mode, DEF, EXACT, LEN>();
+    static_assert(pg_fs_window_never_empty(PG_DEF_MIN_CLOSE, PG_DEF_MIN_PERFECT) && pg_fs_window_never_empty(10, PG_DEF_MIN_PERFECT) &&
+                  PG_DEF_MIN_PERFECT < PG_DEF_MIN_CLOSE && PG_DEF_MIN_PERFECT < 10,
+                  "the short fold step: the window [L - 3, L) of every L >= 8 holds a base, and L > min_perfect at both ends");
     S.depth = rb[0];
     S.jmask[0] = rb[1];
     S.jmask[1] = 0u;
@@ -1657,7 +1704,7 @@
                 Q.first_ok_ = (flags & (flipped ? PG_RF_FIRST_OK_FWD : PG_RF_FIRST_OK_REV)) != 0u;
                 close_bases = e1 > s1 ? e1 - s1 : 0;
                 if (att != 2) {
-                    A.reset();
+                    A.template reset<SF>();
                     S.cap_state = 255;
                     S.nsurv = 0;
                     nsurv_eval = 0;
@@ -1672,9 +1719,9 @@
                 const bool own_grid = att == 0 && !shared_grid;
                 PG_STOP_AT_V(S, 12, true);
                 if (staged)
-                    scan_staged<NB, NS, Id, SM>(S, Q, A, own_grid ? s1 : w1s, s1, e1, w1s, PG_LANE, shared_grid, cr0, cr1, vr);
+                    scan_staged<NB, NS, Id, SM, SF>(S, Q, A, own_grid ? s1 : w1s, s1, e1, w1s, PG_LANE, shared_grid, cr0, cr1, vr);
                 else
-                scan_range<NB, NS, Id, !DEF, SM>(ref, S, Q, A, chr_wo, own_grid ? s1 : w1s, s1, e1, own_grid ? e1 : w1e, ps, pe, w1s, 0u,
+                scan_range<NB, NS, Id, !DEF, SM, SF>(ref, S, Q, A, chr_wo, own_grid ? s1 : w1s, s1, e1, own_grid ? e1 : w1e, ps, pe, w1s, 0u,
                                    PG_LANE, (att == 1 || att == 2 ? 1u : 0u) | shared_grid, cr0, cr1, vr);
                 PG_STOPPED_V(S, true);
                 PG_STOP_AT_V(S, 19, true);
@@ -1684,7 +1731,7 @@
                     nsurv_eval = S.nsurv;
                     Eval<NB, Id> E;
                     PG_DC(S, 0);
-                    evaluate<NB, Id, SE>(S, A, E, PG_LANE);
+                    evaluate<NB, Id, SE, SF>(S, A, E, PG_LANE);
                     PG_STOP_AT_V(S, 20, true);
                     close_max = uni(E.max_len);
                     if (uni(E.n_runs) > 0) {
@@ -1764,7 +1811,7 @@
             auto far_update = [&](int origin, const pg_window *bdw, int qmask) {
                 Eval<NB, Id> E;
                 PG_DC(S, 4);
-                evaluate<NB, Id, SE>(S, A, E, PG_LANE, qmask);
+                evaluate<NB, Id, SE, SF>(S, A, E, PG_LANE, qmask);
                 const int mx = uni(E.max_len);
                 if (mx >= far_max) {
                     far_max = mx;
@@ -1791,7 +1838,7 @@
             if (bd_all && rc[1] != 0u) {
                 const int nbd = (int)rc[1];
                 const pg_window *bd = bd_all + rc[2];
-                A.reset();
+                A.template reset<SF>();
                 S.cap_state = 255;
                 S.nsurv = 0;
                 for (int w = 0; w < nbd; w++) {
@@ -1801,7 +1848,7 @@
                     const int csz = own_chr ? chr_size : chr_size_of<NB>(ref, S, uni(bw.chr_id));
                     const int s = st < 0 ? 0 : st, e = bw.end > csz ? csz : bw.end;
                     far_bases += (e > s ? e - s : 0) + 2 * len;
-                    scan_range<NB, NS, Id, !DEF, SM>(ref, S, Q, A, own_chr ? chr_wo : chr_word_off_of<NB>(ref, S, uni(bw.chr_id)), s, s, e, e, 0, 0, st,
+                    scan_range<NB, NS, Id, !DEF, SM, SF>(ref, S, Q, A, own_chr ? chr_wo : chr_word_off_of<NB>(ref, S, uni(bw.chr_id)), s, s, e, e, 0, 0, st,
                                        (u32)w, PG_LANE, false, unused0, unused1, unused_valid);
                     PG_STOPPED(S);
                 }
@@ -1823,7 +1870,7 @@
                 u32 cacheF = 0u, cacheB = 0u;
                 u32 cache_valid = 0u;
                 int ps = 0, pe = 0, nsurv_eval = 0;
-                A.reset();
+                A.template reset<SF>();
                 S.cap_state = 255;
                 if (k_mri >= 3) S.sf |= 1u;
                 S.nsurv = 0;
@@ -1891,7 +1938,7 @@
                                 PG_STOP_AT(S, 27);
                                 int ring_n[3];
                                 PG_T(S, 7);
-                                fold_candidates<NB, Id, true, SM>(S, Q, A, wb, origin, 0u, total, lane,
+                                fold_candidates<NB, Id, true, SM, SF>(S, Q, A, wb, origin, 0u, total, lane,
                                                               Rings{ true, rs[0], re[0], rs[1], re[1] }, ring_n);
                                 PG_STOPPED(S);
                                 PG_STOP_AT(S, 30);
@@ -1901,7 +1948,7 @@
                                         u64 longm[NB];
 #pragma unroll
                                         for (int k = 0; k < NB; k++) longm[k] = read_lane(S.ringB[r * NB + k], 0);
-                                        fold_tier_b<NB, Id, SM>(S, Q, A, longm, lane);
+                                        fold_tier_b<NB, Id, SM, SF>(S, Q, A, longm, lane);
                                         far_update(origin, nullptr, r == 0 ? 1 : (r == 1 ? 3 : 15));
                                     }
                                     if (far_max + close_max >= len) {
@@ -1922,7 +1969,7 @@
                     int s, e;
                     range_of(span, s, e);
                     if (s < e) {
-                        scan_range<NB, NS, Id, !DEF, SM>(ref, S, Q, A, chr_wo, g0, s, e, emax, ps, pe, origin, 0u, PG_LANE, true,
+                        scan_range<NB, NS, Id, !DEF, SM, SF>(ref, S, Q, A, chr_wo, g0, s, e, emax, ps, pe, origin, 0u, PG_LANE, true,
                                            cacheF, cacheB, cache_valid);
                         PG_STOPPED(S);
                         if (ps < pe) {
```

Measured after the change: 571.6 million reads/s (median of 6 runs). 3.9% higher.
